# navigator8972/vae_assoc

Hardware: AMD Instinct MI355X
Metric: paired-samples/sec (img+jnt assoc-VAE train step) (higher is better)
Workload: dtype bf16

## Files before the change

### vae_assoc_amd/csrc/avae_device.h

```cpp
#pragma once
#include <hip/hip_runtime.h>
#include <math.h>
#include <stdint.h>
#include "../../include/avae.h"

namespace avae {

constexpr int kMaxMod = 4;
constexpr int kThreads = 256;
constexpr int kTileBytesK = 128;
constexpr int kRowAlign = 256;
constexpr int kLatentRows = 16;
constexpr int kAdamRows = 16;
constexpr int kCostHist = 4096;
constexpr int kSumsqThreads = 256;
constexpr int kSumsqMaxBlocks = 256;
constexpr int kSumsqQuads = 8;
inline int sumsq_blocks(long long p_int) {
    const long long quads = p_int / 4, per_block = (long long)kSumsqThreads * kSumsqQuads;
    const long long g = (quads + per_block - 1) / per_block;
    return (int)(g < 1 ? 1 : g > kSumsqMaxBlocks ? kSumsqMaxBlocks : g);
}
inline int sumsq_chain(long long p_int) {
    const long long quads = p_int / 4, per_pass = (long long)kSumsqThreads * sumsq_blocks(p_int);
    return (int)((quads + per_pass - 1) / per_pass);
}

enum Kind : int {
    K_FWD_HIDDEN = 0,
    K_FWD_HEAD = 1,
    K_FWD_OUT_LOSS = 2,
    K_FWD_OUT_STORE = 3,
    K_DGRAD_HIDDEN = 4,
    K_DGRAD_LATENT = 5,
    K_WGRAD = 6,
    K_DGRAD_F32 = 10,
    K_LATENT = 7,
    K_COST = 8,
    K_SERVE_Z = 11,
};

struct WorkItem {
    int kind;
    int M, N, K;
    int lda, ldb;
    int tiles_m, tiles_n;
    int act;
    int ld0, ld1, ldx;
    int nz;
    int binary;
    int ksplit, kchunk;
    int bias_row;
    int bias_ep;
    int kin;
    int tile_off, tile_cnt;
    int slot_base;
    int n_slots;
    int n_mod;
    int bump_step;
    float scale;
    float lambda;
    float inv_bg;
    const void* A;
    const void* B;
    void* out0;
    void* out1;
    void* out2;
    const void* aux0;
    const void* aux1;
    const void* aux2;
    float* partial;
    const float* eps;
    float wts[kMaxMod];
    const void* tail_w;
    void* tail_out;
    const void* tail_aux;
    int tail_mode;
    int tail_n;
    int tail_ldw, tail_ldo, tail_ldx;
    int tail_act;
    int tail_kt;
    int conv;
    const unsigned char* present;
    int present_ld;
};

struct ConvA {
    const void* src;
    const void* consts;
    int M, K;
    int OHW, OW, IH, IW, Cin;
    int k, so, d, pad;
    int src_sb, src_sp;
    int ones;
    unsigned mg_ohw, mg_ow, mg_k, mg_cin;
};
constexpr int kMaxConvA = 12;
constexpr int kMaxItemsPerLaunch = 12;
constexpr int kMaxPf = 4;
struct LaunchArgs {
    int n_items;
    int grid_x;
    int sched;
    int n_pf;
    const void* pf_ptr[4];
    int pf_lines[4];
    const ConvA* conv_tab;
    WorkItem items[kMaxItemsPerLaunch];
};

struct TnItem {
    const void* A;
    const void* B;
    float* out;
    int M, N, K;
    int lda, ldb, ld0;
    int tiles_m, tiles_n;
    int ksplit, kchunk;
    int bias_row;
    int tile_off, tile_cnt;
    int conv;
    void* W; void* Wt;
    int ldw, ldt;
};
constexpr int kMaxTnItems = 32;
constexpr int kTnPieces = 8;
struct TnPiece { unsigned short item, tile_off, cum_end, pad; };
struct DevState;
struct TnLaunchArgs {
    int n_items;
    int grid_x;
    int xcd_group;
    int sched;
    int adam;
    long long d_theta, d_m, d_v;
    float beta1, beta2, eps;
    const DevState* st;
    const ConvA* conv_tab;
    int xcd_pieces;
    TnPiece pieces[8][kTnPieces];
    TnItem items[kMaxTnItems];
};
static_assert(sizeof(TnLaunchArgs) <= 4096, "kernel arguments are passed by value: 4 KiB");

struct alignas(64) SmallDesc {
    const unsigned char* a;
    const unsigned char* b;
    void* out;
    const void* aux;
    int lda, ldb, ld0, ldx;
    int nk;
    int mrem, nrem, xrem;
};
struct alignas(64) TnDesc {
    const unsigned char* a;
    const unsigned char* b;
    float* out;
    void* w;
    void* wt;
    int lda, ldb, ld0, ldw, ldt;
    unsigned ext;
    static constexpr unsigned pack(int nk, int mrem, int nrem) { return (unsigned)nk | (unsigned)(mrem < 64 ? mrem : 64) << 16 | (unsigned)(nrem < 64 ? nrem : 64) << 24; }
};
static_assert(sizeof(SmallDesc) == 64 && sizeof(TnDesc) == 64, "a descriptor is one cache line");
struct DescWarm { const void* lines; int n; };
struct TnDescArgs {
    long long d_theta, d_m, d_v;
    float beta1, beta2, eps;
    const DevState* st;
};
constexpr int kTnDescHead = 8;
static_assert(sizeof(TnDescArgs) <= 64, "a copy of the constants is one line of the table");

struct DevState {
    long long step;
    float last_cost;
    float lr_t;
    float cost_hist[kCostHist];
};

struct ClipState {
    float max_norm;
    int skip_nonfinite;
    long long n_skipped;
    float partial[kSumsqMaxBlocks];
    float norm_hist[kCostHist];
};

struct EmaState {
    float decay;
    int warmup;
    int pad[30];
};
static_assert(sizeof(EmaState) == 128, "the average is line-aligned behind its settings");

struct HyperEntry { float kl, lambda, lr, pad; };
constexpr int kHyperSets = 16;
struct SchedState {
    avae_schedule sched[3];
    float lambda0, lr0;
    HyperEntry tab[kHyperSets];
    float hist[kCostHist][3];
};

__host__ __device__ inline float schedule_value(const avae_schedule& s, long long t) {
#pragma clang fp contract(off)
    long long u = t - 1;
    if (u < 0) u = 0;
    if (s.kind == AVAE_SCHED_PIECEWISE) {
        if (s.period > 0) u %= s.period;
        const int last = s.n_knots - 1;
        if (u <= s.knot_step[0]) return s.knot_value[0];
        if (u >= s.knot_step[last]) return s.knot_value[last];
        int i = 0;
        while (i + 1 < last && u >= s.knot_step[i + 1]) ++i;
        const double v0 = (double)s.knot_value[i], v1 = (double)s.knot_value[i + 1];
        const double f = (double)(u - s.knot_step[i]) / (double)(s.knot_step[i + 1] - s.knot_step[i]);
        return (float)(v0 + (v1 - v0) * f);
    }
    if (s.kind == AVAE_SCHED_EXP) {
        const double e = s.staircase ? (double)(u / s.decay_steps) : (double)u / (double)s.decay_steps;
        return (float)pow((double)s.decay_rate, e);
    }
    return 1.0f;
}

struct AdamItem {
    float* theta;
    float* m;
    float* v;
    const float* g;
    void* W;
    void* Wt;
    int rows, cols;
    int ld, ldt;
    int tiles_r, tiles_c, tile_base;
    int ldw;
    void* Wadj; void* Wf;
    int ldadj, ldf, adj_k, adj_cin;
};

constexpr int kMaxAdamItems = 80;
struct AdamArgs {
    const AdamItem* items;
    int n_items;
    int base[kMaxAdamItems];
    int mode;
    int book;
    float lr, beta1, beta2, eps;
    DevState* st;
    const float* cost_src;
    ClipState* clip;
    int n_partial;
    const EmaState* ema;
    float* avg;
    const float* theta0;
};

struct PrepSeg {
    const float* src; int src_ld;
    int rows, cols;
    float* dst32; int ld32;
    void* dstc; int ldc;
    int tiles_r, tiles_c, tile_base;
    const float* src_in; int in_ld;
    unsigned drop_thr;
    float drop_value, noise_std;
};
struct PrepArgs {
    PrepSeg seg[kMaxMod];
    int n_seg;
    int total_tiles;
    const float* eps_src;
    float* eps_dst;
    int eps_rows, nz, eps_blocks, eps_ld;
    int row_offset;
    unsigned long long seed;
    const DevState* st;
    unsigned long long stream_salt;
    int n_steps, blocks_per_step;
    long long set_stride;
    const unsigned char* pres_src;
    unsigned char* pres_dst;
    int pres_ld;
    int noisy;
    SchedState* sched;
};

struct ReduceSeg { float* dst; const float* src; int n, parts; long long stride; int block_base;
                   int dst_ld;
                   int colsum;
                   int perm_k, perm_cin, perm_cout, perm_ldga, perm_ld; };
constexpr int kMaxReduceSegs = 40;
struct ReduceArgs { ReduceSeg seg[kMaxReduceSegs]; int n_seg; };

struct ConvGeom {
    int B, IH, IW, Cin, OH, OW, k, so, d, pad;
    int src_sb, src_sp;
    int ones;
};
struct GatherSeg {
    ConvGeom g;
    const void* src;
    void* P; int ldp;
    int tiles_r, tiles_c, tile_base;
    int cl, rpt;
};
struct GatherArgs { GatherSeg seg[kMaxMod]; int n_seg; };
struct Col2imSeg {
    ConvGeom g;
    const float* dP; int lddp;
    const void* yprev; int ldy;
    int act;
    void* dA; int lda;
    const float* g0; int nz;
    const void* bias; int bias_ld;
    int tiles_r, tiles_c, tile_base;
// ... 33 lines not shown
void launch_gperm(const GpermArgs& a, int n_blocks, hipStream_t s);
struct RowsumSeg { const void* src; float* part; int ld, rows, cols, cols4, cpow, n_blocks, block_base; };
struct RowsumArgs { RowsumSeg seg[2 * kMaxMod]; int n_seg; };
void launch_rowsum(int compute_dtype, const RowsumArgs& a, int n_blocks, hipStream_t s);

struct ServeSlot {
    const float* z;
    float* out[kMaxMod];
    int rows;
    int pad;
};
struct ServeArgs {
    ServeSlot* slot;
    int n_mod, nz, bucket;
    void* Z[kMaxMod]; int ldz[kMaxMod];
    int blocks_per_mod;
};
void launch_serve(int compute_dtype, const ServeArgs& a, const ServeSlot& call, int n_blocks, hipStream_t s);
struct ServeInMod { const void* w; void* out; int n, ldw, ldo, kt, act, slices; };
struct ServeInArgs {
    ServeSlot call;
    ServeSlot* slot;
    int n_mod, nz, bucket, tiles_m;
    ServeInMod mod[kMaxMod];
};
void launch_serve_in(int compute_dtype, const ServeInArgs& a, int grid_x, hipStream_t s);

void launch_gather(int compute_dtype, const GatherArgs& a, int n_blocks, hipStream_t s);
void launch_col2im(int compute_dtype, const Col2imArgs& a, int n_blocks, hipStream_t s);

constexpr int kScoreRows = kThreads / 64;
struct ScoreLatentArgs {
    const float* mulv[kMaxMod];
    void* Z[kMaxMod]; int ldz[kMaxMod];
    const float* eps; int ld_eps;
    float* out; int k;
    int rows, nz, n_mod;
    int src;
    const unsigned char* present;
};
void launch_score_latent(int compute_dtype, const ScoreLatentArgs& a, hipStream_t s);
struct ScoreRowsArgs {
    const float* xhat; int ld32;
    const float* x; long long ldx;
    float* out; int k;
    int rows, n_in, binary, col;
    int cost;
    int n_mod, n_pair;
    float w[kMaxMod]; float lambda;
    const unsigned char* present; int pa, pb; unsigned absent_bits;
};
void launch_score_rows(const ScoreRowsArgs& a, hipStream_t s);

struct IwLatentArgs {
    const float* mulv;
    const float* eps;
    float* z32;
    void* Z[kMaxMod]; int ldz[kMaxMod]; int n_zdst;
    float* r;
    int rows, kc, k0, K, nz;
    long long row0;
    unsigned long long seed; unsigned draw;
    const unsigned char* present; int pres_ld;
};
void launch_iw_latent(int compute_dtype, const IwLatentArgs& a, hipStream_t s);
struct IwRowsArgs {
    const float* xhat[kMaxMod]; int ldh[kMaxMod];
    const float* x[kMaxMod]; long long ldx[kMaxMod];
    int n_in[kMaxMod], binary[kMaxMod];
    float* ell;
    int n_dec, kc, n_mod;
    const unsigned char* present;
};
void launch_iw_rows(const IwRowsArgs& a, hipStream_t s);
struct IwReduceArgs {
    const float* ell; const float* r;
    float* state;
    float* out; int width;
    int rows, kc, src, n_mod;
    int first, last;
    float log_k;
    const unsigned char* present;
};
void launch_iw_reduce(const IwReduceArgs& a, hipStream_t s);

struct ImputeFuseArgs {
    const float* mulv[kMaxMod];
    unsigned mods;
    const unsigned char* present;
    float* fused;
    float* mu; float* lv;
    float* z32;
    void* Z[kMaxMod]; int ldz[kMaxMod]; int n_zdst;
    int rows, nz, n_mod;
};
void launch_impute_fuse(int compute_dtype, const ImputeFuseArgs& a, hipStream_t s);
struct ImputeAccumArgs {
    const float* xhat[kMaxMod]; int ldh[kMaxMod];
    float* mean[kMaxMod]; float* var[kMaxMod];
    int n_in[kMaxMod];
    int tile0[kMaxMod + 1];
    int col0[kMaxMod];
    float* state; int ld_state;
    int rows, kc, k0, K, n_mod;
};
void launch_impute_accum(const ImputeAccumArgs& a, hipStream_t s);

constexpr int kMaxWorld = 8;
constexpr int kIpcThreads = 256;
struct IpcArgs {
    float* g;
    long long off, granules;
    long long cost_idx;
    int world, rank, wire_bf16, blocks;
    unsigned char* peer[kMaxWorld];
    long long off_flag1, off_flag2;
    long long off_cost;
    long long off_seq;
    long long off_err;
    long long off_slots, slot_stride, off_res;
    unsigned long long timeout_ticks;
};
void launch_ipc_allreduce(const IpcArgs& a, hipStream_t s);
void launch_wire_pack(const float* g, void* wire, long long n, hipStream_t s);
void launch_wire_unpack(float* g, const void* wire, long long n, hipStream_t s);

struct LaunchEvents { hipEvent_t start, stop; };
extern thread_local LaunchEvents t_launch_events;

constexpr int kStampLaunches = 32, kStampBlocks = 1024, kStampWords = 8;

int tile_lds_bytes(int tile_cfg, bool two_c_tiles);
void launch_grouped(int compute_dtype, int tile_cfg, const LaunchArgs& args, int grid_x, int grid_y, int lds_bytes,
                    DevState* st, hipStream_t s, unsigned long long* stamps = nullptr, int launch_id = 0);
void launch_grouped_tn(int compute_dtype, int tile_cfg, const TnLaunchArgs& args, int grid_x, int grid_y, int lds_bytes,
                       DevState* st, hipStream_t s, unsigned long long* stamps = nullptr, int launch_id = 0);
void launch_adam(int compute_dtype, const AdamArgs& a, int n_blocks, hipStream_t s);
void launch_grad_sumsq(const float* g, long long p_int, float* partial, hipStream_t s);
void launch_prep(int compute_dtype, const PrepArgs& a, hipStream_t s);
const void* prep_kernel(int compute_dtype, bool masked, bool noisy, bool sched);
void launch_fill(void* base, int elem_bytes, unsigned bits, long long start, long long stride, int count, hipStream_t s);
void launch_sums(const ReduceArgs& a, int n_blocks, hipStream_t s);
int small_head_lds_bytes();
void launch_small_latb(int compute_dtype, int act, const LaunchArgs& args, int grid_x, int grid_y, int lds_bytes, DevState* st, hipStream_t s,
                       unsigned long long* stamps, int launch_id);
void launch_small_head(int compute_dtype, int act, const LaunchArgs& args, int grid_x, int grid_y, int lds_bytes, hipStream_t s,
                       unsigned long long* stamps, int launch_id);
void launch_small_tn(int compute_dtype, const TnLaunchArgs& args, int grid_x, int grid_y, hipStream_t s, unsigned long long* stamps, int launch_id);
void launch_small_loss(int compute_dtype, const LaunchArgs& args, int grid_x, int grid_y, int lds_bytes, hipStream_t s, unsigned long long* stamps, int launch_id);
void launch_small(int compute_dtype, const LaunchArgs& args, int grid_x, int grid_y, int lds_bytes, hipStream_t s, unsigned long long* stamps, int launch_id);
void launch_small_desc(int compute_dtype, bool dgrad, int act, const SmallDesc* tab, int n_tiles, int lds_bytes, DescWarm warm, hipStream_t s,
                       unsigned long long* stamps, int launch_id);
void launch_small_tn_desc(int compute_dtype, const TnDesc* tab, int n_tiles, DescWarm warm, hipStream_t s, unsigned long long* stamps, int launch_id);
void launch_reduce(const ReduceArgs& a, int n_blocks, hipStream_t s);
void launch_chain2(int compute_dtype, const LaunchArgs& args, int grid_x, int grid_y, int lds_bytes, unsigned* counters, unsigned* err, hipStream_t s);

}
```

### vae_assoc_amd/csrc/avae_host.hip

```cpp
#include "avae_device.h"
#include "avae_complete.h"
#include "avae_retrieve.h"
#include "avae_latent_stats.h"
#include "avae_gmm.h"
#include "avae_embed.h"
#include "avae_aggpost.h"
#include "../../include/avae.h"

#include <dlfcn.h>
#include <sched.h>
#include <unistd.h>

#include <algorithm>
#include <cctype>
#include <cstddef>
#include <cmath>
#include <cstdio>
#include <cstdlib>
#include <cstring>
#include <functional>
#include <map>
#include <mutex>
#include <stdexcept>
#include <string>
// ... 1815 lines not shown
    } else if (md.conv) {
        for (int i = 0; i < 4; ++i) {
            if (md.cdec[i].dense_map) {
                Launch L;
                L.name = "inf_conv_dec_direct"; L.type = 4;
                L.ta.mode = 0;
                ThinSeg t = bd.thin_seg(md.cdec[i], md.cdec[i - 1]);
                t.block_base = 0;
                L.ta.seg[0] = t; L.ta.n_seg = 1;
                L.blocks = rows * t.split;
                inf.launches.push_back(L);
                continue;
            }
            gather1(md.cdec[i], i == 0 ? h->at<void>(md.Z.rm) : h->at<void>(md.cdec[i - 1].Y.rm), "inf_conv_im2col");
            one(bd.conv_fwd(md.cdec[i]), "inf_conv_dec");
        }
        if (!md.cdec[3].dense_map) gather1(md.cdec[4], h->at<void>(md.cdec[3].Y.rm), "inf_conv_im2col");
        one(bd.fwd_out(md, m, false), "inf_out");
    } else {
        for (int k = 0; k < md.L; ++k) one(bd.fwd_hidden(k == 0 ? md.Z : md.D[k - 1], md.dec[k], md.D[k]), "inf_dec");
        one(bd.fwd_out(md, m, false), "inf_out");
    }
    inf.rows = rows;
}

int tname_id(avae_handle* h, const std::string& n) {
    for (size_t i = 0; i < h->tnames.size(); ++i) if (h->tnames[i] == n) return (int)i;
    h->tnames.push_back(n);
    return (int)h->tnames.size() - 1;
}

struct Timed {
    avae_handle* h; hipStream_t s; bool on; hipEvent_t a = nullptr, b = nullptr; int id = 0;
    Timed(avae_handle* h_, hipStream_t s_, const std::string& name) : h(h_), s(s_), on(h_->timing && h_->trecs.size() < 200000) {
        if (!on) return;
        id = tname_id(h, name);
        HIP_OK(hipEventCreate(&a)); HIP_OK(hipEventCreate(&b));
        t_launch_events = LaunchEvents{a, b};
    }
    ~Timed() {
        if (!on) return;
        if (t_launch_events.start) {
            t_launch_events = LaunchEvents{nullptr, nullptr};
            (void)hipEventRecord(a, s); (void)hipEventRecord(b, s);
        }
        h->trecs.push_back(TimingRec{a, b, id});
    }
};

template <typename F> void timed_launch(avae_handle* h, hipStream_t s, const char* name, F&& launch) {
    Timed t(h, s, name);
    launch();
    LAUNCH_OK(name);
}

Launch relocated(const avae_handle* h, const Launch& L0, int j, const HyperEntry* hyper = nullptr) {
    Launch L = L0;
    const unsigned char* lo = h->ws + h->stage_lo;
    const unsigned char* hi = lo + h->stage_bytes;
    const size_t delta = (size_t)j * h->stage_bytes;
    auto fix = [&](auto& ptr) {
        const unsigned char* q = reinterpret_cast<const unsigned char*>(ptr);
        if (q >= lo && q < hi) ptr = reinterpret_cast<std::remove_reference_t<decltype(ptr)>>(const_cast<unsigned char*>(q) + delta);
    };
    for (int i = 0; i < L.args.n_items && L.type == 0; ++i) {
        WorkItem& w = L.args.items[i];
        fix(w.A); fix(w.B); fix(w.out0); fix(w.out1); fix(w.out2); fix(w.aux0); fix(w.aux1); fix(w.aux2); fix(w.eps);
        fix(w.tail_w); fix(w.tail_out); fix(w.tail_aux);
        if (w.present) w.present += (size_t)j * h->pres_set;
        if (hyper && (w.kind == K_LATENT || (w.kind == K_COST && w.bump_step))) w.tail_w = hyper + j;
    }
    for (int i = 0; i < L.targs.n_items && L.type == 0; ++i) { TnItem& t = L.targs.items[i]; fix(t.A); fix(t.B); fix(t.out); }
    for (int i = 0; i < L.ga.n_seg && L.type == 1; ++i) fix(L.ga.seg[i].src);
    L.desc_set = j;
    return L;
}

template <typename D> std::vector<D> deal_to_xcds(const std::vector<D> (&lists)[8]) {
    size_t total = 0;
    for (const auto& l : lists) total += l.size();
    std::vector<D> out(total), spill;
    std::vector<char> set(total, 0);
    for (int p = 0; p < 8; ++p)
        for (size_t i = 0; i < lists[p].size(); ++i) {
            const size_t x = 8 * i + p;
            if (x < total) { out[x] = lists[p][i]; set[x] = 1; } else spill.push_back(lists[p][i]);
        }
    size_t k = 0;
    for (size_t x = 0; x < total; ++x) if (!set[x]) out[x] = spill[k++];
    return out;
}

std::vector<SmallDesc> small_descs(const avae_handle* h, const Launch& L) {
    std::vector<SmallDesc> lists[8];
    const int es = h->es;
    for (int y = 0; y < L.args.n_items; ++y) {
        const WorkItem& w = L.args.items[y];
        if (w.kind != L.args.items[0].kind || w.act != L.args.items[0].act || (w.kind != K_FWD_HIDDEN && w.kind != K_DGRAD_HIDDEN)) return {};
        const int nt = w.tiles_m * w.tiles_n, q = nt >> 3, r = nt & 7;
        for (int part = 0; part < 8; ++part)
            for (int idx = 0; idx < q + (part < r ? 1 : 0); ++idx) {
                const int t = (part < r ? part * (q + 1) : r * (q + 1) + (part - r) * q) + idx;
                const int tm = t / w.tiles_n, tn = t - tm * w.tiles_n, m0 = tm * 32, n0 = tn * 32;
                SmallDesc d{};
                d.a = static_cast<const unsigned char*>(w.A) + (size_t)m0 * w.lda * es;
                d.b = static_cast<const unsigned char*>(w.B) + (size_t)n0 * w.ldb * es;
                d.out = static_cast<unsigned char*>(w.out0) + ((size_t)m0 * w.ld0 + n0) * es;
                d.aux = w.kind == K_DGRAD_HIDDEN ? static_cast<const unsigned char*>(w.aux0) + ((size_t)m0 * w.ldx + n0) * es : nullptr;
                d.lda = w.lda; d.ldb = w.ldb; d.ld0 = w.ld0; d.ldx = w.ldx;
                d.nk = (w.K * es) / kTileBytesK;
                d.mrem = w.M - m0; d.nrem = w.N - n0; d.xrem = w.ldx - n0;
                lists[part].push_back(d);
            }
    }
    return deal_to_xcds(lists);
}

std::vector<TnDesc> tn_descs(const avae_handle* h, const Launch& L) {
    std::vector<TnDesc> lists[8];
    const TnLaunchArgs& a = L.targs;
    const int es = h->es;
    for (int y = 0; y < L.grid_y; ++y)
        for (int x = 0; x < L.grid_x; ++x) {
            const int part = x & 7, idx = x >> 3;
            int entry = y, t = -1;
            if (a.xcd_pieces) {
                int e = 0, lo = 0;
                for (int i = 0; i < kTnPieces; ++i) { const int ce = a.pieces[part][i].cum_end; if (idx >= ce) { e = i + 1; lo = ce; } }
                if (e >= kTnPieces) continue;
                entry = a.pieces[part][e].item; t = a.pieces[part][e].tile_off + idx - lo;
            } else {
                if (entry >= a.n_items) continue;
                const int nt = a.items[entry].tile_cnt, q = nt >> 3, r = nt & 7;
                if (idx >= q + (part < r ? 1 : 0)) continue;
                t = (part < r ? part * (q + 1) : r * (q + 1) + (part - r) * q) + idx + a.items[entry].tile_off;
            }
            const TnItem& w = a.items[entry];
            const int tm = t / w.tiles_n, tn = t - tm * w.tiles_n, m0 = tm * 64, n0 = tn * 64;
            const int nk = (w.K * es) / kTileBytesK;
            if (nk > 65535 || !w.W || !w.Wt) return {};
            TnDesc d{};
            d.a = static_cast<const unsigned char*>(w.A) + (size_t)m0 * es;
            d.b = static_cast<const unsigned char*>(w.B) + (size_t)n0 * es;
            d.out = w.out + (size_t)m0 * w.ld0 + n0;
            d.w = static_cast<unsigned char*>(w.W) + ((size_t)m0 * w.ldw + n0) * es;
            d.wt = static_cast<unsigned char*>(w.Wt) + ((size_t)n0 * w.ldt + m0) * es;
            d.lda = w.lda; d.ldb = w.ldb; d.ld0 = w.ld0; d.ldw = w.ldw; d.ldt = w.ldt;
            d.ext = TnDesc::pack(nk, w.M - m0, w.N - n0);
            lists[part].push_back(d);
        }
    return deal_to_xcds(lists);
}

void build_descriptors(avae_handle* h, hipStream_t s) {
    if (std::getenv("AVAE_NO_DESC")) return;
    std::vector<unsigned char> tab;
    auto add = [&](Launch& L) {
        if (L.type != 0 || !((L.cfg == 7 && !L.tn) || (L.cfg == 12 && L.tn && L.targs.adam))) return;
        const size_t off = tab.size();
        size_t stride = 0;
        int n = 0;
        for (int j = 0; j < kMultiSteps; ++j) {
            const Launch Lj = j == 0 ? L : relocated(h, L, j);
            const size_t at = tab.size();
            if (L.tn) {
                const std::vector<TnDesc> d = tn_descs(h, Lj);
                if (d.empty()) { tab.resize(off); return; }
                const TnDescArgs ca = {L.targs.d_theta, L.targs.d_m, L.targs.d_v, L.targs.beta1, L.targs.beta2, L.targs.eps, L.targs.st};
                tab.resize(at + (kTnDescHead + d.size()) * 64, 0);
                for (int p = 0; p < kTnDescHead; ++p) std::memcpy(tab.data() + at + 64 * p, &ca, sizeof(ca));
                std::memcpy(tab.data() + at + 64 * kTnDescHead, d.data(), d.size() * 64);
                n = (int)d.size();
            } else {
                const std::vector<SmallDesc> d = small_descs(h, Lj);
                if (d.empty()) { tab.resize(off); return; }
                tab.resize(at + d.size() * 64);
                std::memcpy(tab.data() + at, d.data(), d.size() * 64);
                n = (int)d.size();
            }
            stride = tab.size() - at;
        }
        L.desc_n = n; L.desc_off = off; L.desc_stride = stride;
    };
    for (Launch& L : h->plain.fwd) add(L);
    for (Launch& L : h->bwd) add(L);
    for (Launch& L : h->wgrad_adam) add(L);
    if (tab.empty()) return;
    HIP_OK(hipMemcpyAsync(h->desc_buf.ensure(tab.size()), tab.data(), tab.size(), hipMemcpyHostToDevice, s));
    HIP_OK(hipStreamSynchronize(s));
}

template <typename D> const D* desc_of(const avae_handle* h, const Launch& L) {
    return reinterpret_cast<const D*>(h->desc_buf.as<unsigned char>() + L.desc_off + (size_t)L.desc_set * L.desc_stride);
}

DescWarm warm_for(const avae_handle* h, const Launch* next, int next_set) {
    if (!next || next->desc_n == 0 || next_set >= kMultiSteps) return DescWarm{nullptr, 0};
    return DescWarm{h->desc_buf.as<unsigned char>() + next->desc_off + (size_t)next_set * next->desc_stride,
                    next->desc_n + (next->tn ? kTnDescHead : 0)};
}

void dump_launch(const Launch& L) {
    std::fprintf(stderr, "[avae] launch %s type=%d cfg=%d items=%d blocks=%d\n", L.name.c_str(), L.type, L.cfg, L.count, L.blocks);
    if (L.desc_n) std::fprintf(stderr, "        descriptors=%d set=%d\n", L.desc_n, L.desc_set);
    for (int i = 0; i < L.args.n_items && L.type == 0; ++i)
        std::fprintf(stderr, "        item kind=%d M=%d N=%d K=%d lda=%d ldb=%d tiles=%dx%d\n", L.args.items[i].kind, L.args.items[i].M,
                     L.args.items[i].N, L.args.items[i].K, L.args.items[i].lda, L.args.items[i].ldb, L.args.items[i].tiles_m, L.args.items[i].tiles_n);
    for (int i = 0; i < L.ga.n_seg && L.type == 1; ++i)
        std::fprintf(stderr, "        gather B=%d IH=%d Cin=%d OH=%d k=%d so=%d d=%d pad=%d sb=%d sp=%d ones=%d ldp=%d tiles=%dx%d\n", L.ga.seg[i].g.B, L.ga.seg[i].g.IH,
                     L.ga.seg[i].g.Cin, L.ga.seg[i].g.OH, L.ga.seg[i].g.k, L.ga.seg[i].g.so, L.ga.seg[i].g.d, L.ga.seg[i].g.pad, L.ga.seg[i].g.src_sb, L.ga.seg[i].g.src_sp,
                     L.ga.seg[i].g.ones, L.ga.seg[i].ldp, L.ga.seg[i].tiles_r, L.ga.seg[i].tiles_c);
    for (int i = 0; i < L.ca.n_seg && L.type == 2; ++i)
        std::fprintf(stderr, "        col2im B=%d IH=%d Cin=%d OH=%d k=%d lddp=%d lda=%d g0=%p tiles=%dx%d\n", L.ca.seg[i].g.B, L.ca.seg[i].g.IH, L.ca.seg[i].g.Cin,
                     L.ca.seg[i].g.OH, L.ca.seg[i].g.k, L.ca.seg[i].lddp, L.ca.seg[i].lda, (const void*)L.ca.seg[i].g0, L.ca.seg[i].tiles_r, L.ca.seg[i].tiles_c);
}

void run_launch(avae_handle* h, const Launch& L, hipStream_t s, unsigned long long* stamps, int stamp, DescWarm warm = DescWarm{nullptr, 0}) {
    Timed t(h, s, L.name);
    if (L.type == 1) launch_gather(h->cfg.compute_dtype, L.ga, L.blocks, s);
    else if (L.type == 2) launch_col2im(h->cfg.compute_dtype, L.ca, L.blocks, s);
    else if (L.type == 3) launch_reduce(L.ra, L.blocks, s);
    else if (L.type == 4) launch_thin(h->cfg.compute_dtype, L.ta, L.blocks, s);
    else if (L.type == 5) launch_colsum(L.ra, L.blocks, s);
    else if (L.type == 6) launch_wadj(h->cfg.compute_dtype, L.wa, L.blocks, s);
    else if (L.type == 7) launch_gperm(L.gp, L.blocks, s);
    else if (L.type == 8) launch_rowsum(h->cfg.compute_dtype, L.rs, L.blocks, s);
    else if (L.type == 9) launch_sums(L.ra, L.blocks, s);
    else if (L.cfg == 13) launch_chain2(h->cfg.compute_dtype, L.args, L.grid_x, L.grid_y, L.lds, h->at<unsigned>(h->off_chain), h->at<unsigned>(h->off_chain) + kMaxMod * 64, s);
    else if (L.cfg == 11) launch_small_head(h->cfg.compute_dtype, L.lean_act, L.args, L.grid_x, L.grid_y, L.lds, s, stamps, stamp);
    else if (L.cfg == 10) launch_small_latb(h->cfg.compute_dtype, L.lean_act, L.args, L.grid_x, L.grid_y, L.lds, h->state(), s, stamps, stamp);
    else if (L.cfg == 9) launch_small_loss(h->cfg.compute_dtype, L.args, L.grid_x, L.grid_y, L.lds, s, stamps, stamp);
    else if (L.cfg == 7 && L.desc_n) launch_small_desc(h->cfg.compute_dtype, L.args.items[0].kind == K_DGRAD_HIDDEN, L.args.items[0].act, desc_of<SmallDesc>(h, L), L.desc_n, L.lds, warm, s, stamps, stamp);
    else if (L.cfg == 7) launch_small(h->cfg.compute_dtype, L.args, L.grid_x, L.grid_y, L.lds, s, stamps, stamp);
    else if (L.tn && L.cfg == 12 && L.desc_n) launch_small_tn_desc(h->cfg.compute_dtype, desc_of<TnDesc>(h, L), L.desc_n, warm, s, stamps, stamp);
    else if (L.tn && L.cfg == 12) launch_small_tn(h->cfg.compute_dtype, L.targs, L.grid_x, L.grid_y, s, stamps, stamp);
    else if (L.tn) launch_grouped_tn(h->cfg.compute_dtype, L.cfg, L.targs, L.grid_x, L.grid_y, L.lds, h->state(), s, stamps, stamp);
    else launch_grouped(h->cfg.compute_dtype, L.cfg, L.args, L.grid_x, L.grid_y, L.lds, h->state(), s, stamps, stamp);
    LAUNCH_OK(L.name);
    if (h->debug_sync) {
        dump_launch(L);
        std::fflush(stderr);
        HIP_OK(hipStreamSynchronize(s));
    }
}

bool has_hyper_item(const Launch& L) {
    for (int i = 0; i < L.args.n_items && L.type == 0; ++i)
        if (L.args.items[i].kind == K_LATENT || (L.args.items[i].kind == K_COST && L.args.items[i].bump_step)) return true;
    return false;
}

void run_set(avae_handle* h, const std::vector<Launch>& ls, size_t lo, size_t hi, int j, hipStream_t s, int stamp_base = -1, bool train = false,
             const Launch* after = nullptr, int after_set = 0) {
    unsigned long long* stamps = nullptr;
#ifdef AVAE_STAMPS
    if (stamp_base >= 0) stamps = h->at<unsigned long long>(h->off_stamps);
#endif
    const HyperEntry* hyper = nullptr;
    if (train && h->sched_on) {
        if (!h->sched_buf.p) throw Err("internal error: a schedule is on without its device state");
        if (j < 0 || j >= kHyperSets) throw Err("internal error: staging set outside the schedule table");
        hyper = h->sched_buf.as<SchedState>()->tab;
    }
    for (size_t i = lo; i < hi && i < ls.size(); ++i) {
        const int k = stamp_base + (int)(i - lo);
        const bool last = i + 1 >= hi || i + 1 >= ls.size();
        const DescWarm warm = last ? warm_for(h, after, after_set) : warm_for(h, &ls[i + 1], j);
        if (j == 0 && !(hyper && has_hyper_item(ls[i]))) run_launch(h, ls[i], s, stamps, k, warm);
        else run_launch(h, relocated(h, ls[i], j, hyper), s, stamps, k, warm);
    }
}

void run_launches(avae_handle* h, const std::vector<Launch>& ls, hipStream_t s) { run_set(h, ls, 0, ls.size(), 0, s); }

void run_adam(avae_handle* h, int mode, hipStream_t s, int bucket = -1, bool from_avg = false) {
    AdamArgs a;
    std::memset(&a, 0, sizeof(a));
    int blocks = h->adam_blocks;
    if (bucket < 0) {
        a.items = h->at<AdamItem>(h->off_adam);
        a.n_items = (int)h->adam_items.size();
        if (a.n_items > kMaxAdamItems) throw Err("internal error: too many Adam items");
        for (int i = 0; i < a.n_items; ++i) a.base[i] = h->adam_items[i].tile_base;
    } else {
        a.items = h->at<AdamItem>(h->off_adam_b) + h->adam_first_b[bucket];
        a.n_items = h->adam_count_b[bucket];
        for (int i = 0; i < a.n_items; ++i) a.base[i] = h->adam_items_b[h->adam_first_b[bucket] + i].tile_base;
        blocks = h->adam_blocks_b[bucket];
        if (blocks == 0) return;
    }
    a.book = (bucket <= 0) ? 1 : 0;
    a.mode = mode;
    a.lr = h->cfg.learning_rate; a.beta1 = h->cfg.beta1; a.beta2 = h->cfg.beta2; a.eps = h->cfg.adam_eps;
    a.st = h->state();
    a.cost_src = h->grad() + h->P_int;
    a.clip = (mode == 0 && h->clip_on) ? h->clip_buf.as<ClipState>() : nullptr;
    a.n_partial = sumsq_blocks((long long)h->P_int);
    if (mode == 0 ? h->ema_on : from_avg) {
        if (!h->ema_buf.p) throw Err("internal error: averaging is on without its device state");
        a.ema = h->ema_buf.as<EmaState>(); a.avg = h->ema_avg(); a.theta0 = h->at<float>(h->off_theta);
    }
    Timed t(h, s, mode == 0 ? (bucket < 0 ? "adam" : bucket == 0 ? "adam_dec" : "adam_enc") : "shadow_refresh");
    launch_adam(h->cfg.compute_dtype, a, blocks, s);
    LAUNCH_OK(mode == 0 ? "adam" : "shadow_refresh");
}

void run_grad_sumsq(avae_handle* h, hipStream_t s) {
    ClipState* cs = h->clip_buf.as<ClipState>();
    if (!cs) throw Err("internal error: clipping is on without its device state");
    timed_launch(h, s, "grad_sumsq", [&] { launch_grad_sumsq(h->grad(), (long long)h->P_int, cs->partial, s); });
}

struct PrepIn { const float* const* in = nullptr; const int32_t* in_ld = nullptr; bool corrupt = false; };

PrepArgs new_prep(const avae_handle* h, unsigned long long salt, int row0 = 0) {
    PrepArgs a;
    std::memset(&a, 0, sizeof(a));
    a.row_offset = h->cfg.row_offset + row0; a.seed = h->cfg.seed; a.st = h->state(); a.stream_salt = salt;
    return a;
}

int fill_prep_seg(const avae_handle* h, PrepSeg& g, const float* src, int src_ld, int rows, int cols, const Act& dst, float* dst32,
                  int ld32, int tile_base) {
    g.src = src; g.src_ld = src_ld; g.rows = rows; g.cols = cols;
    g.dst32 = dst32; g.ld32 = ld32;
    g.dstc = h->at<void>(dst.rm); g.ldc = dst.ld;
    g.tiles_r = (rows + 63) / 64; g.tiles_c = (cols + 63) / 64; g.tile_base = tile_base;
    return g.tiles_r * g.tiles_c;
}

void fill_prep_eps(const avae_handle* h, PrepArgs& a, const float* eps, int rows) {
    a.eps_src = eps; a.eps_dst = h->at<float>(h->off_eps); a.eps_rows = rows; a.nz = h->nz; a.eps_ld = h->ld_eps;
    a.eps_blocks = (rows * ((h->nz + 3) / 4) + kThreads - 1) / kThreads;
}

PrepArgs make_prep_batch(avae_handle* h, const float* const* x, const int32_t* x_ld, const float* eps, int rows,
                         unsigned long long salt, int n_steps = 1, const uint8_t* present = nullptr, const PrepIn& pin = PrepIn()) {
    PrepArgs a = new_prep(h, salt);
    int base = 0;
    for (int m = 0; m < h->M; ++m) {
        const Mod& md = h->mods[m];
        PrepSeg& g = a.seg[m];
        base += fill_prep_seg(h, g, x[m], (x_ld && x_ld[m] > 0) ? x_ld[m] : md.n_in, rows, md.n_in, md.X0, h->at<float>(md.X32), md.ld32, base);
        if (pin.in && pin.in[m]) {
            g.src_in = pin.in[m]; g.in_ld = (pin.in_ld && pin.in_ld[m] > 0) ? pin.in_ld[m] : md.n_in;
            a.noisy = 1;
        } else if (pin.corrupt && (h->drop_thr[m] != 0u || h->corr.noise_std[m] > 0.0f)) {
            g.drop_thr = h->drop_thr[m]; g.drop_value = h->corr.drop_value[m]; g.noise_std = h->corr.noise_std[m];
            a.noisy = 1;
        }
    }
    a.n_seg = h->M; a.total_tiles = base;
    fill_prep_eps(h, a, eps, rows);
    a.n_steps = n_steps; a.blocks_per_step = a.total_tiles + a.eps_blocks; a.set_stride = (long long)h->stage_bytes;
    if (present) { a.pres_src = present; a.pres_dst = h->pres_buf.as<unsigned char>(); a.pres_ld = h->M; }
    if (h->sched_on && salt == kTrainSalt) a.sched = h->sched_buf.as<SchedState>();
    return a;
}

void run_prep_batch(avae_handle* h, const float* const* x, const int32_t* x_ld, const float* eps, int rows,
                    unsigned long long salt, hipStream_t s, const uint8_t* present = nullptr, int n_steps = 1, const PrepIn& pin = PrepIn()) {
    const PrepArgs a = make_prep_batch(h, x, x_ld, eps, rows, salt, n_steps, present, pin);
    timed_launch(h, s, "prep", [&] { launch_prep(h->cfg.compute_dtype, a, s); });
}

struct PrepOne {
    const float* src; int src_ld, rows, cols;
    const Act& dst;
    int row0;
    PrepOne(const float* src_, int src_ld_, int rows_, int cols_, const Act& dst_, int row0_ = 0)
        : src(src_), src_ld(src_ld_), rows(rows_), cols(cols_), dst(dst_), row0(row0_) {}
    float* dst32 = nullptr; int ld32 = 0;
    bool eps = false;
    const float* eps_src = nullptr;
    unsigned long long salt = 0;
    PrepOne& with_eps(const float* e, unsigned long long salt_ = 0) { eps = true; eps_src = e; salt = salt_; return *this; }
    const unsigned char* pres_src = nullptr; unsigned char* pres_dst = nullptr; int pres_ld = 0;
};

void run_prep_single(avae_handle* h, const PrepOne& p, hipStream_t s) {
    PrepArgs a = new_prep(h, p.salt, p.row0);
    if (p.pres_src) { a.pres_src = p.pres_src; a.pres_dst = p.pres_dst; a.pres_ld = p.pres_ld; }
    if (p.src || p.pres_src) {
        a.n_seg = 1;
        a.total_tiles = fill_prep_seg(h, a.seg[0], p.src, p.src_ld, p.rows, p.cols, p.dst, p.dst32, p.ld32, 0);
    }
    if (p.eps) fill_prep_eps(h, a, p.eps_src, p.rows);
    launch_prep(h->cfg.compute_dtype, a, s);
    LAUNCH_OK("prep");
}

StepGraph capture(avae_handle* h, const std::function<void(hipStream_t)>& body, bool with_prep = false) {
    StepGraph sg;
    const bool tsave = h->timing;
    h->timing = false;
    HIP_OK(hipStreamBeginCapture(h->cap_stream, hipStreamCaptureModeThreadLocal));
    try { body(h->cap_stream); }
    catch (...) { (void)hipStreamEndCapture(h->cap_stream, &sg.graph); sg.release(); h->timing = tsave; throw; }
    h->timing = tsave;
    HIP_OK(hipStreamEndCapture(h->cap_stream, &sg.graph));
    try {
        if (with_prep) {
            size_t n_root = 0;
            HIP_OK(hipGraphGetRootNodes(sg.graph, nullptr, &n_root));
            if (n_root != 1) throw Err("internal error: the captured step is not a chain");
            HIP_OK(hipGraphGetRootNodes(sg.graph, &sg.prep, &n_root));
            hipGraphNodeType ty;
            HIP_OK(hipGraphNodeGetType(sg.prep, &ty));
            if (ty != hipGraphNodeTypeKernel) throw Err("internal error: the captured step does not start with the staging kernel");
        }
        HIP_OK(hipGraphInstantiate(&sg.exec, sg.graph, nullptr, nullptr, 0));
        if (!with_prep) { HIP_OK(hipGraphDestroy(sg.graph)); sg.graph = nullptr; }
    } catch (...) { sg.release(); throw; }
    return sg;
}

void patch_prep(avae_handle* h, const StepGraph& sg, const float* const* x, const int32_t* x_ld, const float* eps,
                int n_steps, const uint8_t* present, const PrepIn& pin) {
    PrepArgs a = make_prep_batch(h, x, x_ld, eps, h->B, kTrainSalt, n_steps, present, pin);
    void* kp[1] = {&a};
    hipKernelNodeParams np;
    std::memset(&np, 0, sizeof(np));
    np.func = const_cast<void*>(prep_kernel(h->cfg.compute_dtype, present != nullptr, a.noisy != 0, a.sched != nullptr));
    np.gridDim = dim3((a.total_tiles + a.eps_blocks) * n_steps); np.blockDim = dim3(kThreads);
    np.sharedMemBytes = 0; np.kernelParams = kp; np.extra = nullptr;
    HIP_OK(hipGraphExecKernelNodeSetParams(sg.exec, sg.prep, &np));
}

void fill_ones(avae_handle* h, const Act& a, hipStream_t s) {
    if (!a.ones) return;
    const unsigned bits = h->es == 2 ? 0x3F80u : 0x3F800000u;
    launch_fill(h->at<void>(a.rm), h->es, bits, a.width, a.ld, h->B, s);
    LAUNCH_OK("fill");
}

void step_body(avae_handle* h, const std::vector<Launch>& fwd, hipStream_t s, int j, int stamp_base = -1, bool more = false) {
    auto sb = [&](size_t k) { return stamp_base < 0 ? -1 : stamp_base + (int)k; };
    auto first_of = [](const std::vector<Launch>& ls) { return ls.empty() ? nullptr : &ls[0]; };
    const bool fused = !h->wgrad_adam.empty() && !h->clip_on && !h->ema_on;
    run_set(h, fwd, 0, fwd.size(), j, s, stamp_base, true, first_of(h->bwd), j);
    run_set(h, h->bwd, 0, h->bwd.size(), j, s, sb(fwd.size()), true, fused ? first_of(h->wgrad_adam) : nullptr, j);
    if (fused) {
        run_set(h, h->wgrad_adam, 0, h->wgrad_adam.size(), j, s, sb(fwd.size() + h->bwd.size()), true, more ? first_of(fwd) : nullptr, j + 1);
        return;
    }
    run_set(h, h->wgrad, 0, h->wgrad.size(), j, s, sb(fwd.size() + h->bwd.size()), true);
    if (h->clip_on) run_grad_sumsq(h, s);
    run_adam(h, 0, s);
}

void capture_steps(avae_handle* h, StepPlan& p, const uint8_t* present) {
    std::vector<const float*> x0(h->M, h->at<float>(h->mods[0].X32));
    try {
        p.full = capture(h, [&](hipStream_t cs) {
            run_prep_batch(h, x0.data(), nullptr, nullptr, h->B, kTrainSalt, cs, present);
            step_body(h, p.fwd, cs, 0, 0);
        }, true);
        for (int gi = 0; gi < 2; ++gi) p.multi[gi] = capture(h, [&](hipStream_t cs) {
            run_prep_batch(h, x0.data(), nullptr, nullptr, h->B, kTrainSalt, cs, present, kMultiSizes[gi]);
            for (int j = 0; j < kMultiSizes[gi]; ++j) step_body(h, p.fwd, cs, j, -1, j + 1 < kMultiSizes[gi]);
        }, true);
    } catch (...) { p.full.release(); p.multi[0].release(); p.multi[1].release(); throw; }
}

void capture_plan(avae_handle* h, StepPlan& p, const uint8_t* present) {
    try {
        capture_steps(h, p, present);
        p.eval = capture(h, [&](hipStream_t cs) { run_launches(h, p.fwd, cs); run_launch(h, h->cost_only, cs, nullptr, -1); });
    } catch (...) { p.release(); throw; }
}

void init_device(avae_handle* h) {
    hipStream_t s = h->cap_stream;
    HIP_OK(hipMemsetAsync(h->ws, 0, h->ws_bytes, s));
    for (const Mod& md : h->mods) {
        for (int j = 0; j < kMultiSteps; ++j) {
            Act x = md.X0;
            x.rm += (size_t)j * h->stage_bytes;
            fill_ones(h, x, s);
        }
        for (const Act& a : md.E) fill_ones(h, a, s);
        fill_ones(h, md.Z, s);
        for (const Act& a : md.D) fill_ones(h, a, s);
        if (md.conv && md.cdec[3].dense_map) fill_ones(h, md.cdec[3].Y, s);
    }
    build_training_plan(h);
    build_descriptors(h, s);
    HIP_OK(hipMemcpyAsync(h->at<void>(h->off_adam), h->adam_items.data(), h->adam_items.size() * sizeof(AdamItem), hipMemcpyHostToDevice, s));
    HIP_OK(hipMemcpyAsync(h->at<void>(h->off_adam_b), h->adam_items_b.data(), h->adam_items_b.size() * sizeof(AdamItem), hipMemcpyHostToDevice, s));
    {
        static const unsigned char c32_bf16[32] = {0, 0, 0, 0, 0, 0, 0, 0, 0, 0, 0, 0, 0, 0, 0, 0, 0x80, 0x3F};
        static const unsigned char c32_f32[32] = {0, 0, 0, 0, 0, 0, 0, 0, 0, 0, 0, 0, 0, 0, 0, 0, 0, 0, 0x80, 0x3F};
        HIP_OK(hipMemcpyAsync(h->at<void>(h->off_consts), h->es == 2 ? c32_bf16 : c32_f32, 32, hipMemcpyHostToDevice, s));
        if (!h->conv_tab.empty()) {
            const unsigned char* lo = h->ws + h->stage_lo;
            for (const ConvA& c : h->conv_tab)
                if (reinterpret_cast<const unsigned char*>(c.src) >= lo && reinterpret_cast<const unsigned char*>(c.src) < lo + h->stage_bytes * kMultiSteps)
                    throw Err("internal error: an implicit patch matrix on a staged input (not relocatable per step)");
            HIP_OK(hipMemcpyAsync(h->at<void>(h->off_conv_tab), h->conv_tab.data(), h->conv_tab.size() * sizeof(ConvA), hipMemcpyHostToDevice, s));
        }
    }
    size_t off = h->off_inf;
    h->inf_enc.assign(h->M, avae_handle::Inf());
    h->inf_dec.assign(h->M, avae_handle::Inf());
    for (int m = 0; m < h->M; ++m) {
        h->inf_enc[m].dev_off = off; off += ((size_t)h->mods[m].L + 1) * sizeof(WorkItem);
        h->inf_dec[m].dev_off = off; off += ((size_t)h->mods[m].L + 1) * sizeof(WorkItem);
    }
    HIP_OK(hipStreamSynchronize(s));
    if (h->cfg.use_graph) capture_plan(h, h->plain, nullptr);
}

void comm_check_error(avae_handle* h);

void fetch_cost(avae_handle* h, float* cost_host, bool from_state, hipStream_t s) {
    if (!cost_host) return;
    const void* src = from_state ? (const void*)&h->state()->last_cost : (const void*)(h->grad() + h->P_int);
    HIP_OK(hipMemcpyAsync(cost_host, src, sizeof(float), hipMemcpyDeviceToHost, s));
    HIP_OK(hipStreamSynchronize(s));
    comm_check_error(h);
}

void copy_rows(void* dst, size_t dpitch, const void* src, size_t spitch, size_t width, size_t rows, hipStream_t s) {
    HIP_OK(hipMemcpy2DAsync(dst, dpitch, src, spitch, width, rows, hipMemcpyDeviceToDevice, s));
}

hipStream_t on_stream(avae_handle* h, void* stream) {
    hipStream_t s = reinterpret_cast<hipStream_t>(stream);
    if (h->has_last_stream && s != h->last_stream) {
        if (!h->ev_switch) HIP_OK(hipEventCreateWithFlags(&h->ev_switch, hipEventDisableTiming));
        if (hipEventRecord(h->ev_switch, h->last_stream) == hipSuccess) HIP_OK(hipStreamWaitEvent(s, h->ev_switch, 0));
        else (void)hipGetLastError();
    }
    h->last_stream = s; h->has_last_stream = true;
    return s;
}

void check_schedule(const avae_schedule& c, const std::string& who) {
    auto fail = [&](const std::string& what) { throw Err(who + ": " + what); };
    if (c.kind == AVAE_SCHED_NONE) return;
    if (c.kind == AVAE_SCHED_PIECEWISE) {
        if (c.n_knots < 1 || c.n_knots > AVAE_SCHED_MAX_KNOTS)
            fail("n_knots = " + std::to_string(c.n_knots) + " must be in [1, " + std::to_string(AVAE_SCHED_MAX_KNOTS) + "]");
        if (c.period < 0) fail("period = " + std::to_string((long long)c.period) + " must be >= 0");
        for (int i = 0; i < c.n_knots; ++i) {
            if (i == 0 ? c.knot_step[0] < 0 : c.knot_step[i] <= c.knot_step[i - 1])
                fail("knot_step[" + std::to_string(i) + "] = " + std::to_string((long long)c.knot_step[i]) +
                     (i == 0 ? " must be >= 0" : " must be above knot_step[" + std::to_string(i - 1) + "] (strictly increasing)"));
            if (!(c.knot_value[i] >= 0.0f) || std::isinf(c.knot_value[i]))
                fail("knot_value[" + std::to_string(i) + "] must be finite and >= 0");
        }
        if (c.period > 0 && c.knot_step[c.n_knots - 1] >= c.period)
            fail("knot_step[" + std::to_string(c.n_knots - 1) + "] = " + std::to_string((long long)c.knot_step[c.n_knots - 1]) +
                 " must be below period = " + std::to_string((long long)c.period));
        return;
    }
    if (c.kind == AVAE_SCHED_EXP) {
        if (!(c.decay_rate > 0.0f) || std::isinf(c.decay_rate)) fail("decay_rate must be finite and > 0");
        if (c.decay_steps <= 0) fail("decay_steps = " + std::to_string((long long)c.decay_steps) + " must be > 0");
        if (c.staircase != 0 && c.staircase != 1) fail("staircase must be 0 or 1");
        return;
    }
    fail("kind = " + std::to_string(c.kind) + " is none of AVAE_SCHED_NONE, AVAE_SCHED_PIECEWISE, AVAE_SCHED_EXP");
}

avae_schedule canonical_schedule(const avae_schedule& c) {
    avae_schedule o;
    std::memset(&o, 0, sizeof(o));
    o.kind = c.kind;
    if (c.kind == AVAE_SCHED_PIECEWISE) {
        o.n_knots = c.n_knots; o.period = c.period;
        for (int i = 0; i < c.n_knots; ++i) { o.knot_step[i] = c.knot_step[i]; o.knot_value[i] = c.knot_value[i]; }
    } else if (c.kind == AVAE_SCHED_EXP) {
        o.decay_rate = c.decay_rate; o.staircase = c.staircase; o.decay_steps = c.decay_steps;
    }
    return o;
}

template <typename F> int guarded(avae_handle* h, F&& f) {
    if (!h) return 1;
    std::lock_guard<std::mutex> lk(h->mu);
    try {
        DeviceGuard dg(h->cfg.device);
        f();
        return 0;
    } catch (const std::exception& e) {
        h->err = e.what();
        return 2;
    }
}

void master_to_host(avae_handle* h, size_t off, std::vector<float>& host) {
    host.resize(h->P_int);
    HIP_OK(hipDeviceSynchronize());
// ... 385 lines not shown
void stage_and_encode(avae_handle* h, const RowInputs& in, const RowPresence& pres, int r0, int n, bool encode_null,
                      const StageEps* eps, hipStream_t s) {
    for (int m = 0; m < h->M; ++m) {
        if (!in.x[m] && !pres) continue;
        const Mod& md = h->mods[m];
        PrepOne p(in.at(m, r0), in.ld[m], n, md.n_in, md.X0, r0);
        if (eps && m == 0) p.with_eps(eps->src ? eps->src + (size_t)r0 * h->nz : nullptr);
        if (eps) p.salt = eps->salt;
        if (pres) { p.pres_src = pres.src + (size_t)r0 * h->M + m; p.pres_dst = pres.staged + m; p.pres_ld = h->M; }
        run_prep_single(h, p, s);
        if (in.x[m] || encode_null) run_inference(h, m, true, n, s);
    }
}

struct DecodeAll {
    avae_handle* h;
    bool by_mod;
    explicit DecodeAll(avae_handle* h_) : h(h_), by_mod(decode_by_mod(h_)) {}
    template <typename Args> void z_dest(Args& a, float* z32) const {
        if (!by_mod) { a.z32 = z32; return; }
        a.n_zdst = h->M;
        for (int m = 0; m < h->M; ++m) { a.Z[m] = h->at<void>(h->mods[m].Z.rm); a.ldz[m] = h->mods[m].Z.ld; }
    }
    int ld_out32(int m) const { return by_mod ? h->mods[m].ld32 : h->mods[m].n_in; }
    void run(int nd, const float* z, bool stage_z, float* const* dst, bool dst_only, hipStream_t s) const {
        if (by_mod) {
            for (int m = 0; m < h->M; ++m) {
                float* out = dst ? dst[m] : nullptr;
                if (dst_only && !out) continue;
                if (stage_z) { decode_rows(h, m, z, nd, out, s); continue; }
                run_inference(h, m, false, nd, s);
                if (out) copy_out32(h, m, out, nd, s);
            }
            return;
        }
        ServeSlot sl;
        std::memset(&sl, 0, sizeof(sl));
        for (int c0 = 0; c0 < nd; c0 += h->B) {
            sl.z = z + (size_t)c0 * h->nz; sl.rows = std::min(h->B, nd - c0);
            for (int m = 0; m < h->M; ++m)
                sl.out[m] = (dst && dst[m]) ? dst[m] + (size_t)c0 * h->mods[m].n_in : h->at<float>(h->mods[m].out32);
            serve_call(h, serve_plan(h, serve_bucket(h, sl.rows)), sl, s);
        }
    }
};

struct SampleBlocks {
    int K, n_rows, kb;
    SampleBlocks(int K_, int cap) : K(K_), n_rows(K_ >= cap ? 1 : cap / std::max(K_, 1)), kb(K_ >= cap ? cap : K_) {}
    template <typename F> void each(int nj, F&& body) const {
        for (int k0 = 0; k0 < K; k0 += kb) {
            const int kc = std::min(kb, K - k0);
            body(k0, kc, nj * kc);
        }
    }
};

constexpr int kCompleteSizes[3] = {16, 4, 1};

void complete_pass(avae_handle* h, avae_handle::Complete& cp, hipStream_t s) {
    run_launches(h, cp.fwd, s);
    timed_launch(h, s, "complete_out", [&] { launch_complete_out(h->cfg.compute_dtype, cp.args, s); });
    run_launches(h, cp.bwd, s);
    timed_launch(h, s, "complete_update", [&] { launch_complete_update(h->cfg.compute_dtype, cp.args, s); });
}

avae_handle::Complete& complete_plan(avae_handle* h) {
    avae_handle::Complete& cp = h->cmpl;
    if (cp.built) return cp;
    const int B = h->B, M = h->M, nz = h->nz, lddz = (int)rup(nz, 4);
    Bump b;
    const size_t off_call = b.take(sizeof(CompleteCall));
    const size_t off_z = b.take((size_t)B * nz * 4), off_m = b.take((size_t)B * nz * 4), off_v = b.take((size_t)B * nz * 4);
    const size_t off_recon = b.take((size_t)B * M * 4);
    size_t off_dz[kMaxMod] = {0, 0, 0, 0};
    for (int m = 0; m < M; ++m) off_dz[m] = b.take(rup(B, kRowAlign) * (size_t)lddz * 4);
    unsigned char* buf = static_cast<unsigned char*>(cp.buf.ensure(b.off, true));
    CompleteArgs& a = cp.args;
    std::memset(&a, 0, sizeof(a));
    a.call = reinterpret_cast<CompleteCall*>(buf + off_call);
    a.z32 = reinterpret_cast<float*>(buf + off_z); a.m = reinterpret_cast<float*>(buf + off_m); a.v = reinterpret_cast<float*>(buf + off_v);
    a.recon = reinterpret_cast<float*>(buf + off_recon);
    a.beta1 = h->cfg.beta1; a.beta2 = h->cfg.beta2; a.eps = h->cfg.adam_eps;
    a.n_mod = M; a.nz = nz; a.bucket = B;
    for (int m = 0; m < M; ++m) {
        const Mod& md = h->mods[m];
        a.Z[m] = h->at<void>(md.Z.rm); a.ldz[m] = md.Z.ld;
        a.out32[m] = h->at<float>(md.out32); a.ld32[m] = md.ld32;
        a.dO[m] = h->at<void>(md.dO.rm); a.lddo[m] = md.dO.ld;
        a.dz[m] = reinterpret_cast<float*>(buf + off_dz[m]); a.lddz[m] = lddz;
        a.n_in[m] = md.n_in; a.binary[m] = h->cfg.mod[m].binary ? 1 : 0; a.w[m] = h->cfg.mod[m].weight;
    }
    cp.items.clear(); cp.fwd.clear(); cp.bwd.clear();
    Builder bd(h, cp.items, B, false);
    Groups group{h, cp.items};
    int Lmax = 0;
    for (const Mod& md : h->mods) Lmax = std::max(Lmax, md.L);
    for (int k = 0; k < Lmax; ++k)
        group("cmpl_dec" + std::to_string(k + 1), cp.fwd, [&] {
            for (Mod& md : h->mods) if (k < md.L) cp.items.push_back(bd.fwd_hidden(k == 0 ? md.Z : md.D[k - 1], md.dec[k], md.D[k])); });
    group("cmpl_out", cp.fwd, [&] { for (int m = 0; m < M; ++m) cp.items.push_back(bd.fwd_out(h->mods[m], m, false)); });
    group("cmpl_bwd_out", cp.bwd, [&] {
        for (Mod& md : h->mods) cp.items.push_back(bd.dgrad_hidden(md.dO, md.outl, md.D.back(), md.dD.back())); });
    for (int k = Lmax - 1; k >= 1; --k)
        group("cmpl_bwd_dec" + std::to_string(k + 1), cp.bwd, [&] {
            for (Mod& md : h->mods) if (k < md.L) cp.items.push_back(bd.dgrad_hidden(md.dD[k], md.dec[k], md.D[k - 1], md.dD[k - 1])); });
    group("cmpl_bwd_dz", cp.bwd, [&] {
        for (int m = 0; m < M; ++m) {
            const Mod& md = h->mods[m];
            const Dense& d = md.dec[0];
            WorkItem w = gemm_item(K_DGRAD_F32, B, nz, bd.K_of(d.out), h->at<void>(md.dD[0].rm), md.dD[0].ld, h->at<void>(d.W), d.ldw);
            w.out0 = const_cast<float*>(a.dz[m]); w.ld0 = lddz;
            cp.items.push_back(w);
        } });
    if (h->cfg.use_graph) {
        try {
            for (int i = 0; i < 3; ++i)
                cp.g[i] = capture(h, [&](hipStream_t cs) { for (int j = 0; j < kCompleteSizes[i]; ++j) complete_pass(h, cp, cs); });
        } catch (...) { for (StepGraph& g : cp.g) g.release(); throw; }
    }
    cp.built = true;
    return cp;
}

void build_masked(avae_handle* h) {
    if (!h->masked.fwd.empty()) return;
    h->pres_set = (size_t)h->B * h->M;
    unsigned char* pres = static_cast<unsigned char*>(h->pres_buf.ensure(h->pres_set * kMultiSteps, true));
    std::vector<Launch> mf = h->plain.fwd;
    int n_loss = 0, n_latent = 0;
    for (Launch& L : mf) {
        if (L.type != 0 || L.tn) continue;
        bool gated = false;
        for (int i = 0; i < L.args.n_items; ++i) {
            WorkItem& w = L.args.items[i];
            if (w.kind == K_FWD_OUT_LOSS) {
                int m = 0;
                while (m < h->M && w.aux0 != h->at<void>(h->mods[m].X32)) ++m;
                if (m == h->M) throw Err("internal error: a loss item of no modality");
                w.present = pres + m; w.present_ld = h->M;
                gated = true; ++n_loss;
            } else if (w.kind == K_LATENT) {
                w.present = pres; w.present_ld = h->M;
                gated = true; ++n_latent;
            }
        }
        const int c = L.cfg;
        if (gated && !(c == 0 || c == 1 || c == 3 || c == 4 || c == 5 || c == 6 || c == 9))
            throw Err("masked training is not available on this plan: launch " + L.name + " (tile configuration " + std::to_string(c) +
                      ") carries a loss or latent item on a kernel without the presence gate");
    }
    if (n_loss != h->M || n_latent != 1) throw Err("internal error: the masked twin found " + std::to_string(n_loss) + " loss and " +
                                                   std::to_string(n_latent) + " latent items");
    h->masked.fwd.swap(mf);
    if (h->cfg.use_graph) {
        try { capture_plan(h, h->masked, pres); } catch (...) { h->masked.fwd.clear(); throw; }
    }
}

void check_masked_call(avae_handle* h, const char* what, const float* const* x_dev, const uint8_t* present_dev) {
    if (h->cfg.world_size > 1 || h->cfg.use_comm != AVAE_COMM_NONE || h->comm_on)
        throw Err(std::string(what) + ": masked steps run on one replica only (world_size 1, use_comm AVAE_COMM_NONE)");
    if (!x_dev) throw Err(std::string(what) + ": null x_dev");
    if (!present_dev) throw Err(std::string(what) + ": present_dev is null (unmasked calls go through the unmasked entry points)");
}

void check_inputs(avae_handle* h, const char* what, const float* const* x_dev, const float* const* in_dev, const int32_t* in_ld) {
    if (!x_dev) throw Err(std::string(what) + ": null x_dev");
    for (int m = 0; in_dev && m < h->M; ++m) {
        if (!in_dev[m]) continue;
        if (!x_dev[m]) throw Err(std::string(what) + ": in_dev[" + std::to_string(m) + "] is set while x_dev[" + std::to_string(m) + "] is null");
        if (in_ld && in_ld[m] > 0 && in_ld[m] < h->mods[m].n_in)
            throw Err(std::string(what) + ": in_ld[" + std::to_string(m) + "] = " + std::to_string(in_ld[m]) + " is below n_input = " +
                      std::to_string(h->mods[m].n_in));
    }
}

void train_one(avae_handle* h, StepPlan& p, const float* const* x_dev, const int32_t* x_ld, const uint8_t* present, const float* eps_dev,
               const PrepIn& pin, hipStream_t s) {
    if (h->comm_on) {
        run_prep_batch(h, x_dev, x_ld, eps_dev, h->B, kTrainSalt, s, nullptr, 1, pin);
        dp_step(h, 0, s);
        return;
    }
    if (p.full.exec && !h->timing) {
        patch_prep(h, p.full, x_dev, x_ld, eps_dev, 1, present, pin);
        HIP_OK(hipGraphLaunch(p.full.exec, s));
        return;
    }
    run_prep_batch(h, x_dev, x_ld, eps_dev, h->B, kTrainSalt, s, present, 1, pin);
    step_body(h, p.fwd, s, 0);
    if (h->timing) {
        timed_launch(h, s, "_null_kernel", [&] { launch_fill(h->at<void>(h->off_partial), 4, 0u, 0, 1, 1, s); });
    }
}

struct BatchRun {
    const avae_handle* h;
    const float* const* x_dev;
    const int32_t* x_ld;
    const uint8_t* present;
    const float* eps_dev;
    const float* const* in_dev;
    const int32_t* in_ld;
    const float* x[kMaxMod] = {};
    const float* in[kMaxMod] = {};
    const uint8_t* pres = nullptr;
    const float* eps = nullptr;
    PrepIn pin() const { return PrepIn{in, in_ld, true}; }
    void at(int i) {
        for (int m = 0; m < h->M; ++m) {
            const size_t ld = (x_ld && x_ld[m] > 0) ? (size_t)x_ld[m] : (size_t)h->mods[m].n_in;
            x[m] = x_dev[m] ? x_dev[m] + (size_t)i * h->B * ld : nullptr;
            const size_t ldi = (in_ld && in_ld[m] > 0) ? (size_t)in_ld[m] : (size_t)h->mods[m].n_in;
            in[m] = (in_dev && in_dev[m]) ? in_dev[m] + (size_t)i * h->B * ldi : nullptr;
        }
        pres = present ? present + (size_t)i * h->B * h->M : nullptr;
        eps = eps_dev ? eps_dev + (size_t)i * h->B * h->nz : nullptr;
    }
};

template <typename Ready>
int replay_runs(avae_handle* h, StepGraph (&g)[2], BatchRun& b, int n_steps, hipStream_t s, Ready&& ready) {
    int i = 0;
    for (int gi = 0; gi < 2; ++gi)
        for (; i + kMultiSizes[gi] <= n_steps && ready(gi); i += kMultiSizes[gi]) {
            b.at(i);
            patch_prep(h, g[gi], b.x, b.x_ld, b.eps, kMultiSizes[gi], b.pres, b.pin());
            HIP_OK(hipGraphLaunch(g[gi].exec, s));
        }
    return i;
}

void train_steps(avae_handle* h, StepPlan& p, int n_steps, const float* const* x_dev, const int32_t* x_ld, const float* const* in_dev,
                 const int32_t* in_ld, const uint8_t* present, const float* eps_dev, float* cost_host, hipStream_t s) {
    BatchRun b{h, x_dev, x_ld, present, eps_dev, in_dev, in_ld};
    int i = 0;
    if (h->comm_on) {
        if (h->cfg.use_graph && !h->timing)
            i = replay_runs(h, h->g_dpm, b, n_steps, s, [&](int gi) {
                if (h->dp_graph_failed) return false;
                if (h->g_dpm[gi].exec) return true;
                std::vector<const float*> x0(h->M, h->at<float>(h->mods[0].X32));
                try {
                    h->g_dpm[gi] = capture(h, [&](hipStream_t cs) {
                        run_prep_batch(h, x0.data(), nullptr, nullptr, h->B, kTrainSalt, cs, nullptr, kMultiSizes[gi]);
                        for (int j = 0; j < kMultiSizes[gi]; ++j) dp_step(h, j, cs, true);
                    }, true);
                } catch (const std::exception& e) {
                    h->dp_graph_failed = true;
                    (void)hipGetLastError();
                    if (std::getenv("AVAE_DEBUG_DP")) std::fprintf(stderr, "[avae] data-parallel graph capture failed (%s): host-stepped pipeline\n", e.what());
                    return false;
                }
                return true;
            });
        for (; i < n_steps; i += kMultiSteps) {
            const int n = std::min(kMultiSteps, n_steps - i);
            b.at(i);
            run_prep_batch(h, b.x, x_ld, b.eps, h->B, kTrainSalt, s, nullptr, n, b.pin());
            for (int j = 0; j < n; ++j) dp_step(h, j, s);
        }
    } else {
        if (!h->timing) i = replay_runs(h, p.multi, b, n_steps, s, [&](int gi) { return p.multi[gi].exec != nullptr; });
        for (; i < n_steps; ++i) {
            b.at(i);
            train_one(h, p, b.x, x_ld, b.pres, b.eps, b.pin(), s);
        }
    }
    if (h->clip_on) h->clip_steps += n_steps;
    if (h->sched_on) h->sched_steps += n_steps;
    fetch_cost(h, cost_host, true, s);
}

void eval_cost(avae_handle* h, StepPlan& p, const float* const* x_dev, const int32_t* x_ld, const float* const* in_dev, const int32_t* in_ld,
               const uint8_t* present, const float* eps_dev, float* cost_host, hipStream_t s) {
    run_prep_batch(h, x_dev, x_ld, eps_dev, h->B, 0x6576616cull  | (unsigned long long)next_draw(h, eps_dev) << 34, s, present, 1,
                   PrepIn{in_dev, in_ld, false});
    if (p.eval.exec && !h->timing) HIP_OK(hipGraphLaunch(p.eval.exec, s));
    else { run_launches(h, p.fwd, s); run_launch(h, h->cost_only, s, nullptr, -1); }
    fetch_cost(h, cost_host, false, s);
}

void require_live(const avae_handle* h, const char* who) {
    if (h->averaged)
        throw Err(std::string(who) + ": the handle runs on the averaged weights; call avae_use_averaged(h, 0) before training");
}

void ema_to_host(avae_handle* h, std::vector<float>& host) {
    host.resize(h->P_int);
    HIP_OK(hipDeviceSynchronize());
    HIP_OK(hipMemcpy(host.data(), h->ema_avg(), h->P_int * 4, hipMemcpyDeviceToHost));
}
void host_to_ema(avae_handle* h, const std::vector<float>& host) {
    HIP_OK(hipDeviceSynchronize());
    HIP_OK(hipMemcpy(h->ema_avg(), host.data(), h->P_int * 4, hipMemcpyHostToDevice));
}
void ema_from_theta(avae_handle* h) {
    HIP_OK(hipDeviceSynchronize());
    HIP_OK(hipMemcpy(h->ema_avg(), h->at<void>(h->off_theta), h->P_int * 4, hipMemcpyDeviceToDevice));
    HIP_OK(hipDeviceSynchronize());
}

void use_averaged(avae_handle* h, bool on) {
    if (on && !h->ema_on) throw Err("avae_use_averaged: parameter averaging is off (avae_set_ema)");
    if (on == h->averaged) return;
// ... 1487 lines not shown
```

### vae_assoc_amd/csrc/avae_kernels.hip

```cpp
#include "avae_device.h"
#include "avae_complete.h"
#include <hip/hip_ext.h>
#include <stdexcept>
#include "../../include/avae.h"

namespace avae {

typedef __attribute__((ext_vector_type(8))) __bf16 bf16x8;
typedef __attribute__((ext_vector_type(4))) __bf16 bf16x4;
typedef __attribute__((ext_vector_type(4))) float f32x4;
typedef __attribute__((ext_vector_type(4))) unsigned u32x4;


template <typename CT> __device__ __forceinline__ CT to_ct(float v);
template <> __device__ __forceinline__ float to_ct<float>(float v) { return v; }
template <> __device__ __forceinline__ __bf16 to_ct<__bf16>(float v) { return (__bf16)v; }

__device__ __forceinline__ float bf16_bits_to_float(unsigned b) { return __uint_as_float(b << 16); }

template <typename CT> __device__ __forceinline__ void load4(const CT* p, float v[4]);
template <> __device__ __forceinline__ void load4<float>(const float* p, float v[4]) {
    float4 t = *reinterpret_cast<const float4*>(p);
    v[0] = t.x; v[1] = t.y; v[2] = t.z; v[3] = t.w;
}
// ... 1125 lines not shown
                for (int k = 0; k < HALF; ++k) {
                    if (rws[k] < BM) {
#pragma unroll
                        for (int e = 0; e < 4; ++e) {
                            const int d = 4 * qs[k] + e;
                            if (d < nz) {
                                const float dz = Cs[cs_idx<LDC>(rws[k], d)];
                                Zs[cs_idx<LDC>(rws[k], d)] = dz + gm[k][e];
                                Zs[cs_idx<LDC>(rws[k], nz + d)] = __builtin_fmaf(dz, gf[k][e], gl[k][e]);
                            }
                        }
                    }
                }
            }
        }
        lds_barrier();
        if (ts == 0)
            tile_pass<CT, CT, false, false, BM, BN>(Zs, reinterpret_cast<CT*>(w.out0), w.ld0, (const CT*)nullptr, 8,
                                                    M, 2 * nz, m0, 0, [](float c, float, bool) { return c; });
        if (tail_on) { t_src = Zs; t_cols = 2 * nz; t_one = -1; }
      }
    } break;
    case K_SERVE_Z: {
      if constexpr (TAIL) {
        const int nz = w.nz, rows = w.n_slots;
        float* Zs = Cs + BM * LDC;
        const float* zsrc = reinterpret_cast<const float*>(w.aux0);
        for (int i = tid; i < BM * nz; i += NT) {
            const int r = i / nz, d = i - r * nz;
            Zs[cs_idx<LDC>(r, d)] = m0 + r < rows ? zsrc[(size_t)(m0 + r) * nz + d] : 0.0f;
        }
        if (blockIdx.x == 0 && blockIdx.y == 0 && tid == 0) {
            ServeSlot* sp = reinterpret_cast<ServeSlot*>(w.partial);
            sp->z = zsrc; sp->rows = rows;
            sp->out[0] = reinterpret_cast<float*>(w.out0); sp->out[1] = reinterpret_cast<float*>(w.out1);
            sp->out[2] = reinterpret_cast<float*>(w.out2); sp->out[3] = reinterpret_cast<float*>(const_cast<void*>(w.aux1));
        }
        lds_barrier();
        if (tail_on) { t_src = Zs; t_cols = nz; t_one = nz; }
      }
    } break;
    case K_DGRAD_F32:
    case K_WGRAD: {
        float* G = reinterpret_cast<float*>(w.out0);
        tile_pass<float, float, false, false, BM, BN, NT>(Cs, G, w.ld0, (const float*)nullptr, 4, M, N, m0, n0,
            [](float c, float, bool) { return c; });
    } break;
    default: break;
    }
    if (t_src) tail_product(t_src, t_cols, t_one);
    AVAE_STAMP(4)
    AVAE_STAMP_FLUSH()
    return;
    }
    if constexpr (!TN && (NW == 4 || (NW == 8 && BN == 64))) {
        if (w.kind == K_LATENT) latent_item<NW, MASK>(w, t, red);
        else cost_item<NW>(w, st, red);
        AVAE_STAMP(4)
        AVAE_STAMP_FLUSH()
    }
}

template <typename CT, int KIND, int ACT>
__global__ void __launch_bounds__(kThreads) k_small(const LaunchArgs args, unsigned long long* stamps, int launch_id) {
    constexpr int BM = 32, RING = 4, ES = (int)sizeof(CT), NCH = 2;
    constexpr int kStage = 64 * kTileBytesK;
    unsigned char* smem = avae_dyn_smem;
#ifdef AVAE_STAMPS
    unsigned long long sv[kStampWords] = {0, 0, 0, 0, 0, 0, 0, 0};
#endif
    AVAE_STAMP(0)
    const int part = blockIdx.x & 7, idx = blockIdx.x >> 3;
    const WorkItem w = args.items[blockIdx.y];
    asm volatile("" :: "s"(w.A), "s"(w.B), "s"(w.out0), "s"(w.aux0), "s"(w.lda), "s"(w.ldb), "s"(w.K), "s"(w.ld0), "s"(w.ldx));
    int t;
    {
        const int nt = w.tiles_m * w.tiles_n;
        const int q = nt >> 3, r = nt & 7;
        if (idx >= q + (part < r ? 1 : 0)) return;
        t = (part < r ? part * (q + 1) : r * (q + 1) + (part - r) * q) + idx;
    }
    const int tid = threadIdx.x, lane = tid & 63, wave = __builtin_amdgcn_readfirstlane(tid >> 6);
    const int wr = wave >> 1, wc = wave & 1, fr = lane & 15, fq = lane >> 4;
    const int tm = t / w.tiles_n, tn = t - tm * w.tiles_n;
    const int m0 = tm * BM, n0 = tn * 32;
    const int nk = (w.K * ES) / kTileBytesK;
    typedef const __attribute__((address_space(1))) void* gp_t;
    typedef __attribute__((address_space(3))) void* lp_t;
    const int prow = wave * 8 + (lane >> 3), lc = ((lane & 7) ^ ((prow >> 1) & 7)) * 16;
    const unsigned char* srcA = reinterpret_cast<const unsigned char*>(w.A) + (size_t)(m0 + prow) * w.lda * ES + lc;
    const unsigned char* srcB = reinterpret_cast<const unsigned char*>(w.B) + (size_t)(n0 + prow) * w.ldb * ES + lc;
    const int orow = m0 + wr * 16 + fr, ocol = n0 + wc * 16 + 4 * fq;
    typename Quad<CT>::raw yq;
    if constexpr (KIND == 1)
        yq = *reinterpret_cast<const typename Quad<CT>::raw*>(reinterpret_cast<const CT*>(w.aux0) + (size_t)min(orow, w.M - 1) * w.ldx + min(ocol, w.ldx - 4));
#define AVAE_S_DMA(kt, buf)                                                                                             \
    { __builtin_amdgcn_global_load_lds((gp_t)(srcA + (size_t)(kt) * kTileBytesK), (lp_t)(smem + (buf) * kStage + wave * 1024), 16, 0, 0);          \
      __builtin_amdgcn_global_load_lds((gp_t)(srcB + (size_t)(kt) * kTileBytesK), (lp_t)(smem + (buf) * kStage + (4 + wave) * 1024), 16, 0, 0); }
    AVAE_STAMP(1)
    const int npro = nk < RING - 1 ? nk : RING - 1;
    for (int p = 0; p < npro; ++p) AVAE_S_DMA(p, p)
    const int sw0 = (fq ^ (fr >> 1)) * 16;
    const int aoff = (wr * 16 + fr) * kTileBytesK, boff = (32 + wc * 16 + fr) * kTileBytesK;
    f32x4 acc = {0.f, 0.f, 0.f, 0.f};
    int buf = 0;
    for (int kt = 0; kt < nk; ++kt) {
        const int rem = nk - 1 - kt;
        if (rem >= 2) asm volatile("s_waitcnt vmcnt(4)" ::: "memory");
        else if (rem == 1) asm volatile("s_waitcnt vmcnt(2)" ::: "memory");
        else asm volatile("s_waitcnt vmcnt(0)" ::: "memory");
        asm volatile("s_barrier" ::: "memory");
        if (kt == 0) { AVAE_STAMP(2) }
        const unsigned char* Sb = smem + buf * kStage;
        const u32x4 a0 = *reinterpret_cast<const u32x4*>(Sb + aoff + sw0), b0 = *reinterpret_cast<const u32x4*>(Sb + boff + sw0);
        const int fill = buf == 0 ? RING - 1 : buf - 1;
        if (kt + RING - 1 < nk) AVAE_S_DMA(kt + RING - 1, fill)
        const u32x4 a1 = *reinterpret_cast<const u32x4*>(Sb + aoff + (sw0 ^ 64)), b1 = *reinterpret_cast<const u32x4*>(Sb + boff + (sw0 ^ 64));
        mma<CT>(b0, a0, acc);
        mma<CT>(b1, a1, acc);
        buf = buf + 1 == RING ? 0 : buf + 1;
    }
#undef AVAE_S_DMA
    AVAE_STAMP(3)
    if constexpr (KIND == 2) {
        float v[4];
#pragma unroll
        for (int e = 0; e < 4; ++e) v[e] = w.binary ? sigmoidf_(acc[e]) : acc[e];
        if (w.aux2) {
            const ServeSlot* sp = reinterpret_cast<const ServeSlot*>(w.aux2);
            float* dst = sp->out[w.n_mod] + (size_t)orow * w.N + ocol;
            if (orow < sp->rows) {
#pragma unroll
                for (int e = 0; e < 4; ++e) if (ocol + e < w.N) dst[e] = v[e];
            }
        } else if (orow < w.M && ocol < w.N) {
            store_row<float>(reinterpret_cast<float*>(w.out0) + (size_t)orow * w.ld0 + ocol, v, w.N - ocol);
        }
    } else if (orow < w.M && ocol < w.N) {
        float v[4];
#pragma unroll
        for (int e = 0; e < 4; ++e) {
            if constexpr (KIND == 0) v[e] = act_fwd_t<ACT>(acc[e]);
            else v[e] = acc[e] * act_bwd_t<ACT>(quad_elem<CT>(yq, e));
        }
        store_row<CT>(reinterpret_cast<CT*>(w.out0) + (size_t)orow * w.ld0 + ocol, v, w.N - ocol);
    }
    AVAE_STAMP(4)
    AVAE_STAMP_FLUSH()
}

__device__ __forceinline__ unsigned desc_warm(const void* lines, int n, int wave) {
    typedef const __attribute__((address_space(4))) unsigned* cu_t;
    const int i = (blockIdx.x & 7) + 8 * (4 * (blockIdx.x >> 3) + wave);
    return i < n ? *(cu_t)((unsigned long long)lines + 64ull * (unsigned)i) : 0u;
}

template <typename CT, int KIND, int ACT>
__global__ void __launch_bounds__(kThreads) k_small_desc(const SmallDesc* __restrict__ tab, unsigned long long* stamps, int launch_id,
                                                         const void* warm_lines, int warm_n) {
    constexpr int RING = 4, ES = (int)sizeof(CT);
    constexpr int kStage = 64 * kTileBytesK;
    unsigned char* smem = avae_dyn_smem;
#ifdef AVAE_STAMPS
    unsigned long long sv[kStampWords] = {0, 0, 0, 0, 0, 0, 0, 0};
#endif
    AVAE_STAMP(0)
    const SmallDesc d = tab[blockIdx.x];
    const int tid = threadIdx.x, lane = tid & 63, wave = __builtin_amdgcn_readfirstlane(tid >> 6);
    const int wr = wave >> 1, wc = wave & 1, fr = lane & 15, fq = lane >> 4;
    const int nk = d.nk;
    typedef const __attribute__((address_space(1))) void* gp_t;
    typedef __attribute__((address_space(3))) void* lp_t;
    const int prow = wave * 8 + (lane >> 3), lc = ((lane & 7) ^ ((prow >> 1) & 7)) * 16;
    const unsigned char* srcA = d.a + (size_t)prow * d.lda * ES + lc;
    const unsigned char* srcB = d.b + (size_t)prow * d.ldb * ES + lc;
    const int lrow = wr * 16 + fr, lcol = wc * 16 + 4 * fq;
    typename Quad<CT>::raw yq;
    if constexpr (KIND == 1)
        yq = *reinterpret_cast<const typename Quad<CT>::raw*>(reinterpret_cast<const CT*>(d.aux) + (ptrdiff_t)min(lrow, d.mrem - 1) * d.ldx + min(lcol, d.xrem - 4));
#define AVAE_S_DMA(kt, buf)                                                                                             \
    { __builtin_amdgcn_global_load_lds((gp_t)(srcA + (size_t)(kt) * kTileBytesK), (lp_t)(smem + (buf) * kStage + wave * 1024), 16, 0, 0);          \
      __builtin_amdgcn_global_load_lds((gp_t)(srcB + (size_t)(kt) * kTileBytesK), (lp_t)(smem + (buf) * kStage + (4 + wave) * 1024), 16, 0, 0); }
    AVAE_STAMP(1)
    const int npro = nk < RING - 1 ? nk : RING - 1;
    for (int p = 0; p < npro; ++p) AVAE_S_DMA(p, p)
    const unsigned warmed = desc_warm(warm_lines, warm_n, wave);
    const int sw0 = (fq ^ (fr >> 1)) * 16;
    const int aoff = (wr * 16 + fr) * kTileBytesK, boff = (32 + wc * 16 + fr) * kTileBytesK;
    f32x4 acc = {0.f, 0.f, 0.f, 0.f};
    int buf = 0;
    for (int kt = 0; kt < nk; ++kt) {
        const int rem = nk - 1 - kt;
        if (rem >= 2) asm volatile("s_waitcnt vmcnt(4)" ::: "memory");
        else if (rem == 1) asm volatile("s_waitcnt vmcnt(2)" ::: "memory");
        else asm volatile("s_waitcnt vmcnt(0)" ::: "memory");
        asm volatile("s_barrier" ::: "memory");
        if (kt == 0) { AVAE_STAMP(2) }
        const unsigned char* Sb = smem + buf * kStage;
        const u32x4 a0 = *reinterpret_cast<const u32x4*>(Sb + aoff + sw0), b0 = *reinterpret_cast<const u32x4*>(Sb + boff + sw0);
        const int fill = buf == 0 ? RING - 1 : buf - 1;
        if (kt + RING - 1 < nk) AVAE_S_DMA(kt + RING - 1, fill)
        const u32x4 a1 = *reinterpret_cast<const u32x4*>(Sb + aoff + (sw0 ^ 64)), b1 = *reinterpret_cast<const u32x4*>(Sb + boff + (sw0 ^ 64));
        mma<CT>(b0, a0, acc);
        mma<CT>(b1, a1, acc);
        buf = buf + 1 == RING ? 0 : buf + 1;
    }
#undef AVAE_S_DMA
    AVAE_STAMP(3)
    if (lrow < d.mrem && lcol < d.nrem) {
        float v[4];
#pragma unroll
        for (int e = 0; e < 4; ++e) {
            if constexpr (KIND == 0) v[e] = act_fwd_t<ACT>(acc[e]);
            else v[e] = acc[e] * act_bwd_t<ACT>(quad_elem<CT>(yq, e));
        }
        store_row<CT>(reinterpret_cast<CT*>(d.out) + (size_t)lrow * d.ld0 + lcol, v, d.nrem - lcol);
    }
    asm volatile("" :: "s"(warmed));
    AVAE_STAMP(4)
    AVAE_STAMP_FLUSH()
}

thread_local LaunchEvents t_launch_events = {nullptr, nullptr};

#define AVAE_LAUNCH(kernel, grid, block, lds, stream, ...)                                                   \
    do {                                                                                                     \
        if (t_launch_events.start) {                                                                         \
            hipExtLaunchKernelGGL(kernel, grid, block, lds, stream, t_launch_events.start, t_launch_events.stop, 0, __VA_ARGS__); \
            t_launch_events = LaunchEvents{nullptr, nullptr};                                                \
        } else {                                                                                             \
            hipLaunchKernelGGL(kernel, grid, block, lds, stream, __VA_ARGS__);                               \
        }                                                                                                    \
    } while (0)

template <typename K> static void set_max_lds(K kernel) {
    (void)hipFuncSetAttribute(reinterpret_cast<const void*>(kernel), hipFuncAttributeMaxDynamicSharedMemorySize, 160 * 1024);
}

template <typename CT, bool MASK>
__global__ void __launch_bounds__(kThreads) k_small_loss(const LaunchArgs args, unsigned long long* stamps, int launch_id) {
    constexpr int BM = 32, RING = 4, ES = (int)sizeof(CT);
    constexpr int kStage = 64 * kTileBytesK;
    unsigned char* smem = avae_dyn_smem;
    float* red = reinterpret_cast<float*>(smem + RING * kStage);
#ifdef AVAE_STAMPS
    unsigned long long sv[kStampWords] = {0, 0, 0, 0, 0, 0, 0, 0};
#endif
    AVAE_STAMP(0)
    const int part = blockIdx.x & 7, idx = blockIdx.x >> 3;
    const WorkItem w = args.items[blockIdx.y];
    asm volatile("" :: "s"(w.A), "s"(w.B), "s"(w.out0), "s"(w.aux0), "s"(w.lda), "s"(w.ldb), "s"(w.K), "s"(w.ld0), "s"(w.ldx));
    int t;
    {
        const int nt = w.tiles_m * w.tiles_n;
        const int q = nt >> 3, r = nt & 7;
        if (idx >= q + (part < r ? 1 : 0)) return;
        t = (part < r ? part * (q + 1) : r * (q + 1) + (part - r) * q) + idx;
    }
    if (w.kind == K_LATENT) {
        latent_item<4, MASK>(w, t, red);
        AVAE_STAMP(4)
        AVAE_STAMP_FLUSH()
        return;
    }
    const int tid = threadIdx.x, lane = tid & 63, wave = __builtin_amdgcn_readfirstlane(tid >> 6);
    const int wr = wave >> 1, wc = wave & 1, fr = lane & 15, fq = lane >> 4;
    const int tm = t / w.tiles_n, tn = t - tm * w.tiles_n;
    const int m0 = tm * BM, n0 = tn * 32;
    const int nk = (w.K * ES) / kTileBytesK;
    typedef const __attribute__((address_space(1))) void* gp_t;
    typedef __attribute__((address_space(3))) void* lp_t;
    const int prow = wave * 8 + (lane >> 3), lc = ((lane & 7) ^ ((prow >> 1) & 7)) * 16;
    const unsigned char* srcA = reinterpret_cast<const unsigned char*>(w.A) + (size_t)(m0 + prow) * w.lda * ES + lc;
    const unsigned char* srcB = reinterpret_cast<const unsigned char*>(w.B) + (size_t)(n0 + prow) * w.ldb * ES + lc;
    const int orow = m0 + wr * 16 + fr, ocol = n0 + wc * 16 + 4 * fq;
    const f32x4 xq = *reinterpret_cast<const f32x4*>(reinterpret_cast<const float*>(w.aux0) + (size_t)min(orow, w.M - 1) * w.ldx + min(ocol, w.ldx - 4));
    const bool rpres = !MASK || w.present[(size_t)min(orow, w.M - 1) * w.present_ld] != 0;
#define AVAE_S_DMA(kt, buf)                                                                                             \
    { __builtin_amdgcn_global_load_lds((gp_t)(srcA + (size_t)(kt) * kTileBytesK), (lp_t)(smem + (buf) * kStage + wave * 1024), 16, 0, 0);          \
      __builtin_amdgcn_global_load_lds((gp_t)(srcB + (size_t)(kt) * kTileBytesK), (lp_t)(smem + (buf) * kStage + (4 + wave) * 1024), 16, 0, 0); }
    AVAE_STAMP(1)
    const int npro = nk < RING - 1 ? nk : RING - 1;
    for (int p = 0; p < npro; ++p) AVAE_S_DMA(p, p)
    const int sw0 = (fq ^ (fr >> 1)) * 16;
    const int aoff = (wr * 16 + fr) * kTileBytesK, boff = (32 + wc * 16 + fr) * kTileBytesK;
    f32x4 acc = {0.f, 0.f, 0.f, 0.f};
    int buf = 0;
    for (int kt = 0; kt < nk; ++kt) {
        const int rem = nk - 1 - kt;
        if (rem >= 2) asm volatile("s_waitcnt vmcnt(4)" ::: "memory");
        else if (rem == 1) asm volatile("s_waitcnt vmcnt(2)" ::: "memory");
        else asm volatile("s_waitcnt vmcnt(0)" ::: "memory");
        asm volatile("s_barrier" ::: "memory");
        if (kt == 0) { AVAE_STAMP(2) }
        const unsigned char* Sb = smem + buf * kStage;
        const u32x4 a0 = *reinterpret_cast<const u32x4*>(Sb + aoff + sw0), b0 = *reinterpret_cast<const u32x4*>(Sb + boff + sw0);
        const int fill = buf == 0 ? RING - 1 : buf - 1;
        if (kt + RING - 1 < nk) AVAE_S_DMA(kt + RING - 1, fill)
        const u32x4 a1 = *reinterpret_cast<const u32x4*>(Sb + aoff + (sw0 ^ 64)), b1 = *reinterpret_cast<const u32x4*>(Sb + boff + (sw0 ^ 64));
        mma<CT>(b0, a0, acc);
        mma<CT>(b1, a1, acc);
        buf = buf + 1 == RING ? 0 : buf + 1;
    }
#undef AVAE_S_DMA
    AVAE_STAMP(3)
    const float sc = w.scale;
    float csum = 0.0f, v[4];
#pragma unroll
    for (int e = 0; e < 4; ++e) {
        const bool ok = orow < w.M && ocol + e < w.N && rpres;
        float sl, da;
        if (w.binary) loss_bernoulli(acc[e], xq[e], sc, sl, da);
        else loss_gauss(acc[e], xq[e], sc, sl, da);
        csum += ok ? sl : 0.0f;
        v[e] = ok ? da : 0.0f;
    }
    if (orow < w.M && ocol < w.N) store_row<CT>(reinterpret_cast<CT*>(w.out0) + (size_t)orow * w.ld0 + ocol, v, w.N - ocol);
    const float total = block_sum<4>(csum, red);
    if (tid == 0) w.partial[w.slot_base + t] = total;
    AVAE_STAMP(4)
    AVAE_STAMP_FLUSH()
}
void launch_small_loss(int compute_dtype, const LaunchArgs& args, int grid_x, int grid_y, int lds_bytes, hipStream_t s, unsigned long long* stamps, int launch_id) {
    const dim3 grid(grid_x, grid_y), block(kThreads);
    bool masked = false;
    for (int i = 0; i < args.n_items; ++i) masked = masked || args.items[i].present != nullptr;
    if (masked) {
        if (compute_dtype == AVAE_BF16) AVAE_LAUNCH((k_small_loss<__bf16, true>), grid, block, lds_bytes, s, args, stamps, launch_id);
        else AVAE_LAUNCH((k_small_loss<float, true>), grid, block, lds_bytes, s, args, stamps, launch_id);
    } else if (compute_dtype == AVAE_BF16) AVAE_LAUNCH((k_small_loss<__bf16, false>), grid, block, lds_bytes, s, args, stamps, launch_id);
    else AVAE_LAUNCH((k_small_loss<float, false>), grid, block, lds_bytes, s, args, stamps, launch_id);
}

constexpr int kHeadStage = (32 + 64) * kTileBytesK, kHeadImg = 2 * 32 * kTileBytesK;
int small_head_lds_bytes() { return 4 * kHeadStage + kHeadImg + 64; }

template <typename CT> __device__ __forceinline__ void img_put(unsigned char* img, int row, int d, float v) {
    const int b = d * (int)sizeof(CT), bo = b & 127;
    *reinterpret_cast<CT*>(img + (b >> 7) * (32 * kTileBytesK) + row * kTileBytesK + ((((bo >> 4) ^ ((row >> 1) & 7)) << 4) | (bo & 15))) = to_ct<CT>(v);
}

template <typename CT, int ACT>
__global__ void __launch_bounds__(kThreads) k_small_latb(const LaunchArgs args, DevState* st, unsigned long long* stamps, int launch_id) {
    constexpr int RING = 4, ES = (int)sizeof(CT), TSL = ES == 2 ? 2 : 4;
    unsigned char* smem = avae_dyn_smem;
    unsigned char* img = smem + RING * kHeadStage;
    float* red = reinterpret_cast<float*>(img + kHeadImg);
#ifdef AVAE_STAMPS
    unsigned long long sv[kStampWords] = {0, 0, 0, 0, 0, 0, 0, 0};
#endif
    AVAE_STAMP(0)
    const int part = blockIdx.x & 7, idx = blockIdx.x >> 3;
    const WorkItem w = args.items[blockIdx.y];
    asm volatile("" :: "s"(w.A), "s"(w.B), "s"(w.out0), "s"(w.aux2), "s"(w.lda), "s"(w.ldb), "s"(w.K), "s"(w.ld0), "s"(w.tail_w), "s"(w.tail_out), "s"(w.tail_aux));
    int t;
    {
        const int nt = w.tiles_m * w.tiles_n;
        const int q = nt >> 3, r = nt & 7;
        if (idx >= q + (part < r ? 1 : 0)) return;
        t = (part < r ? part * (q + 1) : r * (q + 1) + (part - r) * q) + idx;
    }
    if (w.kind == K_COST) {
        cost_item<4>(w, st, red);
        AVAE_STAMP(4)
        AVAE_STAMP_FLUSH()
        return;
    }
    const int tid = threadIdx.x, lane = tid & 63, wave = __builtin_amdgcn_readfirstlane(tid >> 6);
    const int wr = wave >> 1, wc = wave & 1, fr = lane & 15, fq = lane >> 4;
    const int tm = t / w.tiles_n, ts = t - tm * w.tiles_n;
    const int m0 = tm * 32;
    const int nk = (w.K * ES) / kTileBytesK, nz = w.nz;
    typedef const __attribute__((address_space(1))) void* gp_t;
    typedef __attribute__((address_space(3))) void* lp_t;
    reinterpret_cast<f32x4*>(img)[tid] = f32x4{0.f, 0.f, 0.f, 0.f};
    reinterpret_cast<f32x4*>(img)[tid + kThreads] = f32x4{0.f, 0.f, 0.f, 0.f};
    const int orow = m0 + wr * 16 + fr;
    const int lde = (nz + 3) & ~3;
    const int t_i = wave & 1, t_c0 = (2 * ts + (wave >> 1)) * 32, t_sl = 2 * w.tail_kt;
    const int prow = wave * 8 + (lane >> 3), lc = ((lane & 7) ^ ((prow >> 1) & 7)) * 16;
    const unsigned char* srcA = reinterpret_cast<const unsigned char*>(w.A) + (size_t)(m0 + prow) * w.lda * ES + lc;
    const unsigned char* srcB = reinterpret_cast<const unsigned char*>(w.B) + (size_t)prow * w.ldb * ES + lc;
    const size_t b32 = (size_t)32 * w.ldb * ES;
#define AVAE_H_DMA(kt, buf)                                                                                             \
    { __builtin_amdgcn_global_load_lds((gp_t)(srcA + (size_t)(kt) * kTileBytesK), (lp_t)(smem + (buf) * kHeadStage + wave * 1024), 16, 0, 0);       \
      __builtin_amdgcn_global_load_lds((gp_t)(srcB + (size_t)(kt) * kTileBytesK), (lp_t)(smem + (buf) * kHeadStage + (4 + wave) * 1024), 16, 0, 0); \
      __builtin_amdgcn_global_load_lds((gp_t)(srcB + b32 + (size_t)(kt) * kTileBytesK), (lp_t)(smem + (buf) * kHeadStage + (8 + wave) * 1024), 16, 0, 0); }
    AVAE_STAMP(1)
    const int npro = nk < RING - 1 ? nk : RING - 1;
    for (int p = 0; p < npro; ++p) AVAE_H_DMA(p, p)
    constexpr int kExtra = 6 + 2 * TSL + 2;
    asm volatile("" ::: "memory"); __builtin_amdgcn_sched_barrier(0);
    f32x4 gm[2], gl[2], gf[2];
#pragma unroll
    for (int j = 0; j < 2; ++j) {
        const float* gr = reinterpret_cast<const float*>(w.aux2) + (size_t)min(orow, w.M - 1) * 3 * lde + min(wc * 32 + j * 16 + 4 * fq, lde - 4);
        gm[j] = *reinterpret_cast<const f32x4*>(gr); gl[j] = *reinterpret_cast<const f32x4*>(gr + lde); gf[j] = *reinterpret_cast<const f32x4*>(gr + 2 * lde);
    }
    u32x4 tb[TSL][2];
    typename Quad<CT>::raw ty[2];
#pragma unroll
    for (int j = 0; j < 2; ++j) {
        const unsigned char* pw = reinterpret_cast<const unsigned char*>(w.tail_w) + (size_t)min(t_c0 + 16 * j + fr, w.tail_n - 1) * w.tail_ldw * ES + fq * 16;
#pragma unroll
        for (int sl = 0; sl < TSL; ++sl) tb[sl][j] = *reinterpret_cast<const u32x4*>(pw + (sl < t_sl ? 64 * sl : 0));
        ty[j] = *reinterpret_cast<const typename Quad<CT>::raw*>(reinterpret_cast<const CT*>(w.tail_aux) + (size_t)min(m0 + 16 * t_i + fr, w.M - 1) * w.tail_ldx
                                                                   + min(t_c0 + 16 * j + 4 * fq, w.tail_ldx - 4));
    }
    asm volatile("" ::: "memory"); __builtin_amdgcn_sched_barrier(0);
    const int sw0 = (fq ^ (fr >> 1)) * 16;
    const int aoff = (wr * 16 + fr) * kTileBytesK, boff = (32 + wc * 32 + fr) * kTileBytesK;
    f32x4 acc[2] = {{0.f, 0.f, 0.f, 0.f}, {0.f, 0.f, 0.f, 0.f}};
    int buf = 0;
    for (int kt = 0; kt < nk; ++kt) {
        const int rem = nk - 1 - kt;
        if (kt < npro) {
            if (rem >= 2) asm volatile("s_waitcnt vmcnt(%0)" :: "n"(6 + kExtra) : "memory");
            else if (rem == 1) asm volatile("s_waitcnt vmcnt(%0)" :: "n"(3 + kExtra) : "memory");
            else asm volatile("s_waitcnt vmcnt(%0)" :: "n"(kExtra) : "memory");
        } else {
            if (rem >= 2) asm volatile("s_waitcnt vmcnt(6)" ::: "memory");
            else if (rem == 1) asm volatile("s_waitcnt vmcnt(3)" ::: "memory");
            else asm volatile("s_waitcnt vmcnt(0)" ::: "memory");
        }
        asm volatile("s_barrier" ::: "memory");
        if (kt == 0) { AVAE_STAMP(2) }
        const unsigned char* Sb = smem + buf * kHeadStage;
        const u32x4 a0 = *reinterpret_cast<const u32x4*>(Sb + aoff + sw0);
        const u32x4 b00 = *reinterpret_cast<const u32x4*>(Sb + boff + sw0), b01 = *reinterpret_cast<const u32x4*>(Sb + boff + 16 * kTileBytesK + sw0);
        const int fill = buf == 0 ? RING - 1 : buf - 1;
        if (kt + RING - 1 < nk) AVAE_H_DMA(kt + RING - 1, fill)
        const u32x4 a1 = *reinterpret_cast<const u32x4*>(Sb + aoff + (sw0 ^ 64));
        const u32x4 b10 = *reinterpret_cast<const u32x4*>(Sb + boff + (sw0 ^ 64)), b11 = *reinterpret_cast<const u32x4*>(Sb + boff + 16 * kTileBytesK + (sw0 ^ 64));
        mma<CT>(b00, a0, acc[0]); mma<CT>(b01, a0, acc[1]);
        mma<CT>(b10, a1, acc[0]); mma<CT>(b11, a1, acc[1]);
        buf = buf + 1 == RING ? 0 : buf + 1;
    }
#undef AVAE_H_DMA
    asm volatile("" :: "v"(ty[0]), "v"(ty[1]));
    AVAE_STAMP(3)
    {
        CT* dH = reinterpret_cast<CT*>(w.out0) + (size_t)orow * w.ld0;
        const bool store = ts == 0 && orow < w.M;
        const int lrow = wr * 16 + fr;
#pragma unroll
        for (int j = 0; j < 2; ++j)
#pragma unroll
            for (int e = 0; e < 4; ++e) {
                const int d = wc * 32 + j * 16 + 4 * fq + e;
                if (d < nz) {
                    const float dz = acc[j][e];
                    const float dmu = dz + gm[j][e], dlv = __builtin_fmaf(dz, gf[j][e], gl[j][e]);
                    img_put<CT>(img, lrow, d, dmu);
                    img_put<CT>(img, lrow, nz + d, dlv);
                    if (store) { dH[d] = to_ct<CT>(dmu); dH[nz + d] = to_ct<CT>(dlv); }
                }
            }
    }
    lds_barrier();
    AVAE_STAMP(5)
    {
        const int arow = 16 * t_i + fr;
        f32x4 tacc[1][2] = {{{0.f, 0.f, 0.f, 0.f}, {0.f, 0.f, 0.f, 0.f}}};
#pragma unroll
        for (int sl = 0; sl < TSL; ++sl)
            if (TSL == 2 || sl < t_sl) {
                const u32x4 ta = *reinterpret_cast<const u32x4*>(img + (sl >> 1) * (32 * kTileBytesK) + arow * kTileBytesK + (((fq + 4 * (sl & 1)) ^ ((arow >> 1) & 7)) << 4));
                mma<CT>(tb[sl][0], ta, tacc[0][0]);
                mma<CT>(tb[sl][1], ta, tacc[0][1]);
            }
        regep_store<CT, 1, 2>(tacc, reinterpret_cast<CT*>(w.tail_out), w.tail_ldo, w.M, w.tail_n, m0 + arow, t_c0, lane,
            [&](int, int j, int r, float v) { return v * act_bwd_t<ACT>(quad_elem<CT>(ty[j], r)); });
    }
    AVAE_STAMP(4)
    AVAE_STAMP_FLUSH()
}
template <typename CT, int ACT>
__global__ void __launch_bounds__(kThreads) k_small_head(const LaunchArgs args, unsigned long long* stamps, int launch_id) {
    constexpr int RING = 4, ES = (int)sizeof(CT), TSL = ES == 2 ? 2 : 4, LDM = 68;
    unsigned char* smem = avae_dyn_smem;
    unsigned char* img = smem + RING * kHeadStage;
    float* MV = reinterpret_cast<float*>(smem);
#ifdef AVAE_STAMPS
    unsigned long long sv[kStampWords] = {0, 0, 0, 0, 0, 0, 0, 0};
#endif
    AVAE_STAMP(0)
    const int part = blockIdx.x & 7, idx = blockIdx.x >> 3;
    const WorkItem w = args.items[blockIdx.y];
    asm volatile("" :: "s"(w.A), "s"(w.B), "s"(w.out0), "s"(w.out1), "s"(w.aux0), "s"(w.lda), "s"(w.ldb), "s"(w.K), "s"(w.ld0), "s"(w.tail_w), "s"(w.tail_out));
    int t;
    {
        const int nt = w.tiles_m * w.tiles_n;
        const int q = nt >> 3, r = nt & 7;
        if (idx >= q + (part < r ? 1 : 0)) return;
        t = (part < r ? part * (q + 1) : r * (q + 1) + (part - r) * q) + idx;
    }
    const int tid = threadIdx.x, lane = tid & 63, wave = __builtin_amdgcn_readfirstlane(tid >> 6);
    const int wr = wave >> 1, wc = wave & 1, fr = lane & 15, fq = lane >> 4;
    const int tm = t / w.tiles_n, ts = t - tm * w.tiles_n;
    const int m0 = tm * 32;
    const int nk = (w.K * ES) / kTileBytesK, nz = w.nz;
    typedef const __attribute__((address_space(1))) void* gp_t;
    typedef __attribute__((address_space(3))) void* lp_t;
    reinterpret_cast<f32x4*>(img)[tid] = f32x4{0.f, 0.f, 0.f, 0.f};
    reinterpret_cast<f32x4*>(img)[tid + kThreads] = f32x4{0.f, 0.f, 0.f, 0.f};
    const int zrow = tid >> 3, zg = tid & 7;
    const f32x4 ev = *reinterpret_cast<const f32x4*>(reinterpret_cast<const float*>(w.aux0) + (size_t)min(m0 + zrow, w.M - 1) * w.ldx + min(4 * zg, w.ldx - 4));
    const int t_i = wave & 1, t_c0 = (2 * ts + (wave >> 1)) * 32, t_sl = 2 * w.tail_kt;
    u32x4 tb[TSL][2];
#pragma unroll
    for (int j = 0; j < 2; ++j) {
        const unsigned char* pw = reinterpret_cast<const unsigned char*>(w.tail_w) + (size_t)min(t_c0 + 16 * j + fr, w.tail_n - 1) * w.tail_ldw * ES + fq * 16;
#pragma unroll
        for (int sl = 0; sl < TSL; ++sl) if (TSL == 2 || sl < t_sl) tb[sl][j] = *reinterpret_cast<const u32x4*>(pw + 64 * sl);
    }
    const int prow = wave * 8 + (lane >> 3), lc = ((lane & 7) ^ ((prow >> 1) & 7)) * 16;
    const unsigned char* srcA = reinterpret_cast<const unsigned char*>(w.A) + (size_t)(m0 + prow) * w.lda * ES + lc;
    const unsigned char* srcB = reinterpret_cast<const unsigned char*>(w.B) + (size_t)prow * w.ldb * ES + lc;
    const size_t b32 = (size_t)32 * w.ldb * ES;
#define AVAE_H_DMA(kt, buf)                                                                                             \
    { __builtin_amdgcn_global_load_lds((gp_t)(srcA + (size_t)(kt) * kTileBytesK), (lp_t)(smem + (buf) * kHeadStage + wave * 1024), 16, 0, 0);       \
      __builtin_amdgcn_global_load_lds((gp_t)(srcB + (size_t)(kt) * kTileBytesK), (lp_t)(smem + (buf) * kHeadStage + (4 + wave) * 1024), 16, 0, 0); \
      __builtin_amdgcn_global_load_lds((gp_t)(srcB + b32 + (size_t)(kt) * kTileBytesK), (lp_t)(smem + (buf) * kHeadStage + (8 + wave) * 1024), 16, 0, 0); }
    AVAE_STAMP(1)
    const int npro = nk < RING - 1 ? nk : RING - 1;
    for (int p = 0; p < npro; ++p) AVAE_H_DMA(p, p)
    const int sw0 = (fq ^ (fr >> 1)) * 16;
    const int aoff = (wr * 16 + fr) * kTileBytesK, boff = (32 + wc * 32 + fr) * kTileBytesK;
    f32x4 acc[2] = {{0.f, 0.f, 0.f, 0.f}, {0.f, 0.f, 0.f, 0.f}};
    int buf = 0;
    for (int kt = 0; kt < nk; ++kt) {
        const int rem = nk - 1 - kt;
        if (rem >= 2) asm volatile("s_waitcnt vmcnt(6)" ::: "memory");
        else if (rem == 1) asm volatile("s_waitcnt vmcnt(3)" ::: "memory");
        else asm volatile("s_waitcnt vmcnt(0)" ::: "memory");
        asm volatile("s_barrier" ::: "memory");
        if (kt == 0) { AVAE_STAMP(2) }
        const unsigned char* Sb = smem + buf * kHeadStage;
        const u32x4 a0 = *reinterpret_cast<const u32x4*>(Sb + aoff + sw0);
        const u32x4 b00 = *reinterpret_cast<const u32x4*>(Sb + boff + sw0), b01 = *reinterpret_cast<const u32x4*>(Sb + boff + 16 * kTileBytesK + sw0);
        const int fill = buf == 0 ? RING - 1 : buf - 1;
        if (kt + RING - 1 < nk) AVAE_H_DMA(kt + RING - 1, fill)
        const u32x4 a1 = *reinterpret_cast<const u32x4*>(Sb + aoff + (sw0 ^ 64));
        const u32x4 b10 = *reinterpret_cast<const u32x4*>(Sb + boff + (sw0 ^ 64)), b11 = *reinterpret_cast<const u32x4*>(Sb + boff + 16 * kTileBytesK + (sw0 ^ 64));
        mma<CT>(b00, a0, acc[0]); mma<CT>(b01, a0, acc[1]);
        mma<CT>(b10, a1, acc[0]); mma<CT>(b11, a1, acc[1]);
        buf = buf + 1 == RING ? 0 : buf + 1;
    }
#undef AVAE_H_DMA
    lds_barrier();
    AVAE_STAMP(3)
    {
        const int orow = m0 + wr * 16 + fr, lrow = wr * 16 + fr;
        float* mulv = reinterpret_cast<float*>(w.out0) + (size_t)orow * w.ld0;
        const bool store = ts == 0 && orow < w.M;
#pragma unroll
        for (int j = 0; j < 2; ++j) {
            const int c0 = wc * 32 + j * 16 + 4 * fq;
            *reinterpret_cast<f32x4*>(MV + lrow * LDM + c0) = acc[j];
            if (store) {
#pragma unroll
                for (int e = 0; e < 4; ++e) if (c0 + e < 2 * nz) mulv[c0 + e] = acc[j][e];
            }
        }
    }
    lds_barrier();
    AVAE_STAMP(5)
    {
        CT* Z = reinterpret_cast<CT*>(w.out1) + (size_t)(m0 + zrow) * w.ld1;
        const bool store = ts == 0 && m0 + zrow < w.M;
#pragma unroll
        for (int e = 0; e < 4; ++e) {
            const int d = 4 * zg + e;
            if (d < nz) {
                const float z = __builtin_fmaf(fexp(0.5f * MV[zrow * LDM + nz + d]), ev[e], MV[zrow * LDM + d]);
                img_put<CT>(img, zrow, d, z);
                if (store) Z[d] = to_ct<CT>(z);
            }
        }
        if (tid < 32) img_put<CT>(img, tid, nz, 1.0f);
    }
    lds_barrier();
    AVAE_STAMP_EP(6)
    {
        const int arow = 16 * t_i + fr;
        f32x4 tacc[1][2] = {{{0.f, 0.f, 0.f, 0.f}, {0.f, 0.f, 0.f, 0.f}}};
#pragma unroll
        for (int sl = 0; sl < TSL; ++sl)
            if (TSL == 2 || sl < t_sl) {
                const u32x4 ta = *reinterpret_cast<const u32x4*>(img + (sl >> 1) * (32 * kTileBytesK) + arow * kTileBytesK + (((fq + 4 * (sl & 1)) ^ ((arow >> 1) & 7)) << 4));
                mma<CT>(tb[sl][0], ta, tacc[0][0]);
                mma<CT>(tb[sl][1], ta, tacc[0][1]);
            }
        regep_store<CT, 1, 2>(tacc, reinterpret_cast<CT*>(w.tail_out), w.tail_ldo, w.M, w.tail_n, m0 + arow, t_c0, lane,
            [&](int, int, int, float v) { return act_fwd_t<ACT>(v); });
    }
    AVAE_STAMP(4)
    AVAE_STAMP_FLUSH()
}
void launch_small_head(int compute_dtype, int act, const LaunchArgs& args, int grid_x, int grid_y, int lds_bytes, hipStream_t s,
                       unsigned long long* stamps, int launch_id) {
    const dim3 grid(grid_x, grid_y), block(kThreads);
#define K_HEAD_B(A) k_small_head<__bf16, A>
#define K_HEAD_F(A) k_small_head<float, A>
    if (compute_dtype == AVAE_BF16) {
        switch (act) {
            case AVAE_ACT_RELU: AVAE_LAUNCH((K_HEAD_B(AVAE_ACT_RELU)), grid, block, lds_bytes, s, args, stamps, launch_id); break;
            case AVAE_ACT_SOFTPLUS: AVAE_LAUNCH((K_HEAD_B(AVAE_ACT_SOFTPLUS)), grid, block, lds_bytes, s, args, stamps, launch_id); break;
            case AVAE_ACT_SIGMOID: AVAE_LAUNCH((K_HEAD_B(AVAE_ACT_SIGMOID)), grid, block, lds_bytes, s, args, stamps, launch_id); break;
            case AVAE_ACT_TANH: AVAE_LAUNCH((K_HEAD_B(AVAE_ACT_TANH)), grid, block, lds_bytes, s, args, stamps, launch_id); break;
            default: AVAE_LAUNCH((K_HEAD_B(AVAE_ACT_IDENTITY)), grid, block, lds_bytes, s, args, stamps, launch_id); break;
        }
    } else {
        switch (act) {
            case AVAE_ACT_RELU: AVAE_LAUNCH((K_HEAD_F(AVAE_ACT_RELU)), grid, block, lds_bytes, s, args, stamps, launch_id); break;
            case AVAE_ACT_SOFTPLUS: AVAE_LAUNCH((K_HEAD_F(AVAE_ACT_SOFTPLUS)), grid, block, lds_bytes, s, args, stamps, launch_id); break;
            case AVAE_ACT_SIGMOID: AVAE_LAUNCH((K_HEAD_F(AVAE_ACT_SIGMOID)), grid, block, lds_bytes, s, args, stamps, launch_id); break;
            case AVAE_ACT_TANH: AVAE_LAUNCH((K_HEAD_F(AVAE_ACT_TANH)), grid, block, lds_bytes, s, args, stamps, launch_id); break;
            default: AVAE_LAUNCH((K_HEAD_F(AVAE_ACT_IDENTITY)), grid, block, lds_bytes, s, args, stamps, launch_id); break;
        }
    }
#undef K_HEAD_B
#undef K_HEAD_F
}
void launch_small_latb(int compute_dtype, int act, const LaunchArgs& args, int grid_x, int grid_y, int lds_bytes, DevState* st, hipStream_t s,
                       unsigned long long* stamps, int launch_id) {
    const dim3 grid(grid_x, grid_y), block(kThreads);
#define K_LATB_B(A) k_small_latb<__bf16, A>
#define K_LATB_F(A) k_small_latb<float, A>
    if (compute_dtype == AVAE_BF16) {
        switch (act) {
            case AVAE_ACT_RELU: AVAE_LAUNCH((K_LATB_B(AVAE_ACT_RELU)), grid, block, lds_bytes, s, args, st, stamps, launch_id); break;
            case AVAE_ACT_SOFTPLUS: AVAE_LAUNCH((K_LATB_B(AVAE_ACT_SOFTPLUS)), grid, block, lds_bytes, s, args, st, stamps, launch_id); break;
            case AVAE_ACT_SIGMOID: AVAE_LAUNCH((K_LATB_B(AVAE_ACT_SIGMOID)), grid, block, lds_bytes, s, args, st, stamps, launch_id); break;
            case AVAE_ACT_TANH: AVAE_LAUNCH((K_LATB_B(AVAE_ACT_TANH)), grid, block, lds_bytes, s, args, st, stamps, launch_id); break;
            default: AVAE_LAUNCH((K_LATB_B(AVAE_ACT_IDENTITY)), grid, block, lds_bytes, s, args, st, stamps, launch_id); break;
        }
    } else {
        switch (act) {
            case AVAE_ACT_RELU: AVAE_LAUNCH((K_LATB_F(AVAE_ACT_RELU)), grid, block, lds_bytes, s, args, st, stamps, launch_id); break;
            case AVAE_ACT_SOFTPLUS: AVAE_LAUNCH((K_LATB_F(AVAE_ACT_SOFTPLUS)), grid, block, lds_bytes, s, args, st, stamps, launch_id); break;
            case AVAE_ACT_SIGMOID: AVAE_LAUNCH((K_LATB_F(AVAE_ACT_SIGMOID)), grid, block, lds_bytes, s, args, st, stamps, launch_id); break;
            case AVAE_ACT_TANH: AVAE_LAUNCH((K_LATB_F(AVAE_ACT_TANH)), grid, block, lds_bytes, s, args, st, stamps, launch_id); break;
            default: AVAE_LAUNCH((K_LATB_F(AVAE_ACT_IDENTITY)), grid, block, lds_bytes, s, args, st, stamps, launch_id); break;
        }
    }
#undef K_LATB_B
#undef K_LATB_F
}

#ifdef AVAE_STAMPS
#define AVAE_SV sv
#else
#define AVAE_SV nullptr
#endif
template <typename CT, bool ADAM, typename F>
__device__ __forceinline__ void small_tn_tile(const TnDesc& d, const TnDescArgs& ca, F&& behind_prologue, unsigned char* smem, unsigned long long* sv) {
    constexpr int BM = 64, RING = 4, ES = (int)sizeof(CT), EPR = kTileBytesK / ES, NCH = 4;
    constexpr int kStage = 2 * BM * kTileBytesK;
    const int tid = threadIdx.x, lane = tid & 63, wave = __builtin_amdgcn_readfirstlane(tid >> 6);
    const int wr = wave >> 1, wc = wave & 1, fr = lane & 15, fq = lane >> 4;
    const int nk = d.ext & 0xFFFF, mrem = (d.ext >> 16) & 0xFF, nrem = d.ext >> 24;
    typedef const __attribute__((address_space(1))) void* gp_t;
    typedef __attribute__((address_space(3))) void* lp_t;
    const unsigned char* src[NCH];
    size_t kadv[NCH];
#pragma unroll
    for (int c = 0; c < NCH; ++c) {
        const int r = (c * 4 + wave) * 8 + (lane >> 3);
        const bool is_a = c < 2;
        const int rr = is_a ? r : r - BM, sub = rr / EPR, k = rr - sub * EPR;
        const int lc = (lane & 7) ^ tn_swz<CT>(k);
        const size_t ld_b = (size_t)(is_a ? d.lda : d.ldb) * ES;
        kadv[c] = (size_t)EPR * ld_b;
        src[c] = (is_a ? d.a : d.b) + (size_t)k * ld_b + (size_t)sub * kTileBytesK + lc * 16;
    }
#define AVAE_T_DMA(kt, buf)                                                                                             \
    { _Pragma("unroll") for (int c = 0; c < NCH; ++c)                                                                   \
        __builtin_amdgcn_global_load_lds((gp_t)(src[c] + (size_t)(kt) * kadv[c]), (lp_t)(smem + (buf) * kStage + (c * 4 + wave) * 1024), 16, 0, 0); }
    int offA[2], offB[2];
#pragma unroll
    for (int i = 0; i < 2; ++i) { offA[i] = tn_frag_off<CT>(wr * 32 + i * 16, lane); offB[i] = BM * kTileBytesK + tn_frag_off<CT>(wc * 32 + i * 16, lane); }
    AVAE_STAMP(1)
    const int npro = nk < RING - 1 ? nk : RING - 1;
    for (int p = 0; p < npro; ++p) AVAE_T_DMA(p, p)
    const float lr_t = behind_prologue();
    const int c4 = (tid & 15) * 4;
    f32x4 pth[4], pmm[4], pvv[4];
    auto fetch_state = [&]() {
#pragma unroll
        for (int k = 0; k < 4; ++k) {
            const int lrow = (tid >> 4) + 16 * k;
            const bool ok = lrow < mrem && c4 < nrem;
            const float* gp = d.out + (size_t)(ok ? lrow : 0) * d.ld0 + (ok ? c4 : 0);
            pth[k] = *reinterpret_cast<const f32x4*>(gp + ca.d_theta);
            pmm[k] = *reinterpret_cast<const f32x4*>(gp + ca.d_m);
            pvv[k] = *reinterpret_cast<const f32x4*>(gp + ca.d_v);
        }
    };
    f32x4 acc[2][2];
#pragma unroll
    for (int i = 0; i < 2; ++i)
#pragma unroll
        for (int j = 0; j < 2; ++j) acc[i][j] = f32x4{0.f, 0.f, 0.f, 0.f};
    int buf = 0;
    for (int kt = 0; kt < nk; ++kt) {
        const int rem = nk - 1 - kt;
        if (rem >= 2) asm volatile("s_waitcnt vmcnt(8)" ::: "memory");
        else if (rem == 1) asm volatile("s_waitcnt vmcnt(4)" ::: "memory");
        else asm volatile("s_waitcnt vmcnt(0)" ::: "memory");
        asm volatile("s_barrier" ::: "memory");
        if (kt == 0) { AVAE_STAMP(2) }
        const unsigned char* Sb = smem + buf * kStage;
        u32x4 a0[2], b0[2], a1[2], b1[2];
#pragma unroll
        for (int i = 0; i < 2; ++i) { a0[i] = tn_frag<CT>(Sb, offA[i], 0); b0[i] = tn_frag<CT>(Sb, offB[i], 0); }
        const int fill = buf == 0 ? RING - 1 : buf - 1;
        if (kt + RING - 1 < nk) AVAE_T_DMA(kt + RING - 1, fill)
#pragma unroll
        for (int i = 0; i < 2; ++i) { a1[i] = tn_frag<CT>(Sb, offA[i], 1); b1[i] = tn_frag<CT>(Sb, offB[i], 1); }
        if constexpr (sizeof(CT) == 2) { tn_wait_lds(); tn_frags_ready(a0); tn_frags_ready(b0); tn_frags_ready(a1); tn_frags_ready(b1); }
#pragma unroll
        for (int i = 0; i < 2; ++i)
#pragma unroll
            for (int j = 0; j < 2; ++j) mma<CT>(b0[j], a0[i], acc[i][j]);
#pragma unroll
        for (int i = 0; i < 2; ++i)
#pragma unroll
            for (int j = 0; j < 2; ++j) mma<CT>(b1[j], a1[i], acc[i][j]);
        buf = buf + 1 == RING ? 0 : buf + 1;
    }
#undef AVAE_T_DMA
    AVAE_STAMP(3)
    if constexpr (!ADAM) {
#pragma unroll
        for (int i = 0; i < 2; ++i) {
            const int row = wr * 32 + i * 16 + fr;
#pragma unroll
            for (int j = 0; j < 2; ++j) {
                const int col = wc * 32 + j * 16 + 4 * fq;
                if (row < mrem && col < nrem) {
                    const float g[4] = {acc[i][j][0], acc[i][j][1], acc[i][j][2], acc[i][j][3]};
                    store_row<float>(d.out + (size_t)row * d.ld0 + col, g, nrem - col);
                }
            }
        }
    } else {
        constexpr int LDT = 65;
        float* T = reinterpret_cast<float*>(smem);
        fetch_state();
        lds_barrier();
#pragma unroll
        for (int i = 0; i < 2; ++i)
#pragma unroll
            for (int j = 0; j < 2; ++j)
#pragma unroll
                for (int e = 0; e < 4; ++e) T[(wr * 32 + i * 16 + fr) * LDT + wc * 32 + j * 16 + 4 * fq + e] = acc[i][j][e];
        lds_barrier();
        const float omb1 = 1.0f - ca.beta1, omb2 = 1.0f - ca.beta2;
        const int r4 = (tid & 15) * 4;
        float g[4][4], th[4][4], m[4][4], v[4][4];
#pragma unroll
        for (int k = 0; k < 4; ++k) {
            const int r = (tid >> 4) + 16 * k;
#pragma unroll
            for (int e = 0; e < 4; ++e) { g[k][e] = T[r * LDT + c4 + e]; th[k][e] = pth[k][e]; m[k][e] = pmm[k][e]; v[k][e] = pvv[k][e]; }
#pragma unroll
            for (int e = 0; e < 4; ++e) adam_update(g[k][e], m[k][e], v[k][e], th[k][e], omb1, omb2, lr_t, ca.eps);
#pragma unroll
            for (int e = 0; e < 4; ++e) T[r * LDT + c4 + e] = th[k][e];
        }
        const bool full = mrem >= BM && nrem >= BM;
        auto store_group = [&](int k, float* gp, CT* wp) {
            store4<float>(gp, g[k]);
            store4<float>(gp + ca.d_theta, th[k]); store4<float>(gp + ca.d_m, m[k]); store4<float>(gp + ca.d_v, v[k]);
            store4<CT>(wp, th[k]);
        };
        if (full) {
#pragma unroll
            for (int k = 0; k < 4; ++k) {
                const int lrow = (tid >> 4) + 16 * k;
                store_group(k, d.out + (size_t)lrow * d.ld0 + c4, reinterpret_cast<CT*>(d.w) + (size_t)lrow * d.ldw + c4);
            }
        } else {
#pragma unroll
            for (int k = 0; k < 4; ++k) {
                const int lrow = (tid >> 4) + 16 * k;
                float* gp = d.out + (size_t)lrow * d.ld0 + c4;
                CT* wp = reinterpret_cast<CT*>(d.w) + (size_t)lrow * d.ldw + c4;
                const int nv = nrem - c4;
                if (lrow < mrem && nv >= 4) {
                    store_group(k, gp, wp);
                } else if (lrow < mrem && nv > 0) {
#pragma unroll
                    for (int e = 0; e < 3; ++e) if (e < nv) {
                        gp[e] = g[k][e]; gp[ca.d_theta + e] = th[k][e]; gp[ca.d_m + e] = m[k][e]; gp[ca.d_v + e] = v[k][e]; wp[e] = to_ct<CT>(th[k][e]);
                    }
                    asm volatile("; partial quad" ::: "memory");
                }
            }
        }
        lds_barrier();
#pragma unroll
        for (int k = 0; k < 4; ++k) {
            const int cc = (tid >> 4) + 16 * k;
            float t[4];
#pragma unroll
            for (int e = 0; e < 4; ++e) t[e] = T[(r4 + e) * LDT + cc];
// ... 1962 lines not shown
```

Baseline: 4.987 million.

## Drive loss, head and latent-backward kernels from precomputed per-tile records

Extends the descriptor-table scheme to the loss (cfg 9), forward head (cfg 11) and latent-backward (cfg 10) launches. The host precomputes a 128-byte record per tile holding base pointers, strides and remainders, dealt across XCDs. Each block reads its record instead of decoding WorkItems and tile indices, and warms the next launch's records behind its DMA prologue. This is meant to cut per-block setup latency in these small, latency-bound kernels. It adds table memory, warm-line logic for paired lines, and separate paths for the masked and non-plain variants, which strip the records.

```diff
diff --git a/vae_assoc_amd/csrc/avae_device.h b/vae_assoc_amd/csrc/avae_device.h
--- a/vae_assoc_amd/csrc/avae_device.h
+++ b/vae_assoc_amd/csrc/avae_device.h
@@ -163,6 +163,42 @@
     static constexpr unsigned pack(int nk, int mrem, int nrem) { return (unsigned)nk | (unsigned)(mrem < 64 ? mrem : 64) << 16 | (unsigned)(nrem < 64 ? nrem : 64) << 24; }
 };
 static_assert(sizeof(SmallDesc) == 64 && sizeof(TnDesc) == 64, "a descriptor is one cache line");
+struct alignas(128) LossRec {
+    const unsigned char* a;
+    const unsigned char* b;
+    void* out;
+    const float* x;
+    float* slot;
+    int lda, ldb, ld0, ldx;
+    int nk;
+    int mrem, nrem, xrem;
+    float scale;
+    int binary;
+    int item, tile;
+    int pad_[10];
+};
+struct alignas(128) HeadRec {
+    const unsigned char* a;
+    const unsigned char* b;
+    void* out0;
+    void* out1;
+    const float* aux;
+    const unsigned char* tail_w;
+    void* tail_out;
+    const void* tail_aux;
+    int lda, ldb, ld0, ld1, ldx;
+    int tail_ldw, tail_ldo, tail_ldx;
+    int nk, nz;
+    int mrem;
+    int tail_n;
+    unsigned tk;
+    int item;
+    int pad_[2];
+    static constexpr unsigned pack(int tail_kt, int ts) { return (unsigned)tail_kt | (unsigned)ts << 8; }
+};
+static_assert(sizeof(LossRec) == 128 && sizeof(HeadRec) == 128, "a head or loss record is two cache lines");
+static_assert(sizeof(LaunchArgs) + 64 <= 4096, "the record kernels pass LaunchArgs by value behind their leading arguments: 4 KiB");
+constexpr int kWarmPairs = 1 << 30;
 struct DescWarm { const void* lines; int n; };
 struct TnDescArgs {
     long long d_theta, d_m, d_v;
@@ -502,6 +538,12 @@
 void launch_small_desc(int compute_dtype, bool dgrad, int act, const SmallDesc* tab, int n_tiles, int lds_bytes, DescWarm warm, hipStream_t s,
                        unsigned long long* stamps, int launch_id);
 void launch_small_tn_desc(int compute_dtype, const TnDesc* tab, int n_tiles, DescWarm warm, hipStream_t s, unsigned long long* stamps, int launch_id);
+void launch_loss_rec(int compute_dtype, const LossRec* tab, int n_recs, int lds_bytes, DescWarm warm, const LaunchArgs& args, hipStream_t s,
+                     unsigned long long* stamps, int launch_id);
+void launch_head_rec(int compute_dtype, int act, const HeadRec* tab, int n_recs, int lds_bytes, DescWarm warm, hipStream_t s,
+                     unsigned long long* stamps, int launch_id);
+void launch_latb_rec(int compute_dtype, int act, const HeadRec* tab, int n_recs, int lds_bytes, DescWarm warm, DevState* st, const LaunchArgs& args,
+                     hipStream_t s, unsigned long long* stamps, int launch_id);
 void launch_reduce(const ReduceArgs& a, int n_blocks, hipStream_t s);
 void launch_chain2(int compute_dtype, const LaunchArgs& args, int grid_x, int grid_y, int lds_bytes, unsigned* counters, unsigned* err, hipStream_t s);
 
diff --git a/vae_assoc_amd/csrc/avae_host.hip b/vae_assoc_amd/csrc/avae_host.hip
--- a/vae_assoc_amd/csrc/avae_host.hip
+++ b/vae_assoc_amd/csrc/avae_host.hip
@@ -1991,18 +1991,104 @@
     return deal_to_xcds(lists);
 }
 
+template <typename F> void tiles_of_part(const WorkItem& w, int part, F&& f) {
+    const int nt = w.tiles_m * w.tiles_n, q = nt >> 3, r = nt & 7;
+    for (int idx = 0; idx < q + (part < r ? 1 : 0); ++idx) f((part < r ? part * (q + 1) : r * (q + 1) + (part - r) * q) + idx);
+}
+
+std::vector<LossRec> loss_recs(const avae_handle* h, const Launch& L) {
+    std::vector<LossRec> lists[8];
+    const int es = h->es;
+    for (int y = 0; y < L.args.n_items; ++y) {
+        const WorkItem& w = L.args.items[y];
+        if ((w.kind != K_FWD_OUT_LOSS && w.kind != K_LATENT) || w.present || w.conv > 0 || w.bias_ep) return {};
+        for (int part = 0; part < 8; ++part)
+            tiles_of_part(w, part, [&](int t) {
+                LossRec d{};
+                d.item = -1;
+                if (w.kind == K_LATENT) { d.item = y; d.tile = t; lists[part].push_back(d); return; }
+                const int tm = t / w.tiles_n, tn = t - tm * w.tiles_n, m0 = tm * 32, n0 = tn * 32;
+                d.a = static_cast<const unsigned char*>(w.A) + (size_t)m0 * w.lda * es;
+                d.b = static_cast<const unsigned char*>(w.B) + (size_t)n0 * w.ldb * es;
+                d.out = static_cast<unsigned char*>(w.out0) + ((size_t)m0 * w.ld0 + n0) * es;
+                d.x = static_cast<const float*>(w.aux0) + (size_t)m0 * w.ldx + n0;
+                d.slot = w.partial + w.slot_base + t;
+                d.lda = w.lda; d.ldb = w.ldb; d.ld0 = w.ld0; d.ldx = w.ldx;
+                d.nk = (w.K * es) / kTileBytesK;
+                d.mrem = w.M - m0; d.nrem = w.N - n0; d.xrem = w.ldx - n0;
+                d.scale = w.scale; d.binary = w.binary;
+                lists[part].push_back(d);
+            });
+    }
+    return deal_to_xcds(lists);
+}
+
+std::vector<HeadRec> head_recs(const avae_handle* h, const Launch& L) {
+    std::vector<HeadRec> lists[8];
+    const int es = h->es;
+    const bool bwd = L.cfg == 10;
+    for (int y = 0; y < L.args.n_items; ++y) {
+        const WorkItem& w = L.args.items[y];
+        const bool cost = bwd && w.kind == K_COST;
+        if (!cost && (w.kind != (bwd ? K_DGRAD_LATENT : K_FWD_HEAD) || w.tail_mode != (bwd ? 2 : 1) || w.tail_act != L.lean_act)) return {};
+        if (!cost && (w.present || w.conv > 0 || w.bias_ep || w.tail_kt < 1 || w.tail_kt > 2)) return {};
+        for (int part = 0; part < 8; ++part)
+            tiles_of_part(w, part, [&](int t) {
+                HeadRec d{};
+                d.item = -1;
+                if (cost) { d.item = y; lists[part].push_back(d); return; }
+                const int tm = t / w.tiles_n, ts = t - tm * w.tiles_n, m0 = tm * 32;
+                d.a = static_cast<const unsigned char*>(w.A) + (size_t)m0 * w.lda * es;
+                d.b = static_cast<const unsigned char*>(w.B);
+                d.tail_w = static_cast<const unsigned char*>(w.tail_w);
+                d.tail_out = static_cast<unsigned char*>(w.tail_out) + (size_t)m0 * w.tail_ldo * es;
+                if (bwd) {
+                    d.out0 = static_cast<unsigned char*>(w.out0) + (size_t)m0 * w.ld0 * es;
+                    d.aux = static_cast<const float*>(w.aux2) + (size_t)m0 * 3 * ((w.nz + 3) & ~3);
+                    d.tail_aux = static_cast<const unsigned char*>(w.tail_aux) + (size_t)m0 * w.tail_ldx * es;
+                } else {
+                    d.out0 = static_cast<float*>(w.out0) + (size_t)m0 * w.ld0;
+                    d.out1 = static_cast<unsigned char*>(w.out1) + (size_t)m0 * w.ld1 * es;
+                    d.aux = static_cast<const float*>(w.aux0) + (size_t)m0 * w.ldx;
+                }
+                d.lda = w.lda; d.ldb = w.ldb; d.ld0 = w.ld0; d.ld1 = w.ld1; d.ldx = w.ldx;
+                d.tail_ldw = w.tail_ldw; d.tail_ldo = w.tail_ldo; d.tail_ldx = w.tail_ldx;
+                d.nk = (w.K * es) / kTileBytesK; d.nz = w.nz;
+                d.mrem = w.M - m0; d.tail_n = w.tail_n;
+                d.tk = HeadRec::pack(w.tail_kt, ts);
+                lists[part].push_back(d);
+            });
+    }
+    return deal_to_xcds(lists);
+}
+
+bool two_line_records(const Launch& L) { return L.type == 0 && !L.tn && (L.cfg == 9 || L.cfg == 10 || L.cfg == 11); }
+
 void build_descriptors(avae_handle* h, hipStream_t s) {
     if (std::getenv("AVAE_NO_DESC")) return;
     std::vector<unsigned char> tab;
     auto add = [&](Launch& L) {
-        if (L.type != 0 || !((L.cfg == 7 && !L.tn) || (L.cfg == 12 && L.tn && L.targs.adam))) return;
+        if (L.type != 0 || !((L.cfg == 7 && !L.tn) || (L.cfg == 12 && L.tn && L.targs.adam) || two_line_records(L))) return;
+        tab.resize((tab.size() + 127) & ~(size_t)127);
         const size_t off = tab.size();
         size_t stride = 0;
         int n = 0;
+        auto put = [&](const auto& d) {
+            if (d.empty()) { tab.resize(off); return false; }
+            const size_t at = tab.size(), bytes = d.size() * sizeof(d[0]);
+            tab.resize(at + bytes);
+            std::memcpy(tab.data() + at, d.data(), bytes);
+            n = (int)d.size();
+            return true;
+        };
         for (int j = 0; j < kMultiSteps; ++j) {
             const Launch Lj = j == 0 ? L : relocated(h, L, j);
             const size_t at = tab.size();
-            if (L.tn) {
+            if (L.cfg == 9) {
+                if (!put(loss_recs(h, Lj))) return;
+            } else if (L.cfg == 10 || L.cfg == 11) {
+                if (!put(head_recs(h, Lj))) return;
+            } else if (L.tn) {
                 const std::vector<TnDesc> d = tn_descs(h, Lj);
                 if (d.empty()) { tab.resize(off); return; }
                 const TnDescArgs ca = {L.targs.d_theta, L.targs.d_m, L.targs.d_v, L.targs.beta1, L.targs.beta2, L.targs.eps, L.targs.st};
@@ -2035,13 +2121,13 @@
 
 DescWarm warm_for(const avae_handle* h, const Launch* next, int next_set) {
     if (!next || next->desc_n == 0 || next_set >= kMultiSteps) return DescWarm{nullptr, 0};
-    return DescWarm{h->desc_buf.as<unsigned char>() + next->desc_off + (size_t)next_set * next->desc_stride,
-                    next->desc_n + (next->tn ? kTnDescHead : 0)};
+    const int lines = two_line_records(*next) ? 2 * next->desc_n | kWarmPairs : next->desc_n + (next->tn ? kTnDescHead : 0);
+    return DescWarm{h->desc_buf.as<unsigned char>() + next->desc_off + (size_t)next_set * next->desc_stride, lines};
 }
 
 void dump_launch(const Launch& L) {
     std::fprintf(stderr, "[avae] launch %s type=%d cfg=%d items=%d blocks=%d\n", L.name.c_str(), L.type, L.cfg, L.count, L.blocks);
-    if (L.desc_n) std::fprintf(stderr, "        descriptors=%d set=%d\n", L.desc_n, L.desc_set);
+    if (L.desc_n) std::fprintf(stderr, two_line_records(L) ? "        records=%d set=%d\n" : "        descriptors=%d set=%d\n", L.desc_n, L.desc_set);
     for (int i = 0; i < L.args.n_items && L.type == 0; ++i)
         std::fprintf(stderr, "        item kind=%d M=%d N=%d K=%d lda=%d ldb=%d tiles=%dx%d\n", L.args.items[i].kind, L.args.items[i].M,
                      L.args.items[i].N, L.args.items[i].K, L.args.items[i].lda, L.args.items[i].ldb, L.args.items[i].tiles_m, L.args.items[i].tiles_n);
@@ -2066,6 +2152,9 @@
     else if (L.type == 8) launch_rowsum(h->cfg.compute_dtype, L.rs, L.blocks, s);
     else if (L.type == 9) launch_sums(L.ra, L.blocks, s);
     else if (L.cfg == 13) launch_chain2(h->cfg.compute_dtype, L.args, L.grid_x, L.grid_y, L.lds, h->at<unsigned>(h->off_chain), h->at<unsigned>(h->off_chain) + kMaxMod * 64, s);
+    else if (L.cfg == 11 && L.desc_n) launch_head_rec(h->cfg.compute_dtype, L.lean_act, desc_of<HeadRec>(h, L), L.desc_n, L.lds, warm, s, stamps, stamp);
+    else if (L.cfg == 10 && L.desc_n) launch_latb_rec(h->cfg.compute_dtype, L.lean_act, desc_of<HeadRec>(h, L), L.desc_n, L.lds, warm, h->state(), L.args, s, stamps, stamp);
+    else if (L.cfg == 9 && L.desc_n) launch_loss_rec(h->cfg.compute_dtype, desc_of<LossRec>(h, L), L.desc_n, L.lds, warm, L.args, s, stamps, stamp);
     else if (L.cfg == 11) launch_small_head(h->cfg.compute_dtype, L.lean_act, L.args, L.grid_x, L.grid_y, L.lds, s, stamps, stamp);
     else if (L.cfg == 10) launch_small_latb(h->cfg.compute_dtype, L.lean_act, L.args, L.grid_x, L.grid_y, L.lds, h->state(), s, stamps, stamp);
     else if (L.cfg == 9) launch_small_loss(h->cfg.compute_dtype, L.args, L.grid_x, L.grid_y, L.lds, s, stamps, stamp);
@@ -2090,7 +2179,7 @@
 }
 
 void run_set(avae_handle* h, const std::vector<Launch>& ls, size_t lo, size_t hi, int j, hipStream_t s, int stamp_base = -1, bool train = false,
-             const Launch* after = nullptr, int after_set = 0) {
+             const Launch* after = nullptr, int after_set = 0, bool records2 = true) {
     unsigned long long* stamps = nullptr;
 #ifdef AVAE_STAMPS
     if (stamp_base >= 0) stamps = h->at<unsigned long long>(h->off_stamps);
@@ -2105,8 +2194,11 @@
         const int k = stamp_base + (int)(i - lo);
         const bool last = i + 1 >= hi || i + 1 >= ls.size();
         const DescWarm warm = last ? warm_for(h, after, after_set) : warm_for(h, &ls[i + 1], j);
-        if (j == 0 && !(hyper && has_hyper_item(ls[i]))) run_launch(h, ls[i], s, stamps, k, warm);
-        else run_launch(h, relocated(h, ls[i], j, hyper), s, stamps, k, warm);
+        const bool strip = !records2 && ls[i].desc_n && two_line_records(ls[i]);
+        if (j == 0 && !(hyper && has_hyper_item(ls[i])) && !strip) { run_launch(h, ls[i], s, stamps, k, warm); continue; }
+        Launch L = relocated(h, ls[i], j, hyper);
+        if (strip) L.desc_n = 0;
+        run_launch(h, L, s, stamps, k, warm);
     }
 }
 
@@ -2278,7 +2370,8 @@
     auto first_of = [](const std::vector<Launch>& ls) { return ls.empty() ? nullptr : &ls[0]; };
     const bool fused = !h->wgrad_adam.empty() && !h->clip_on && !h->ema_on;
     run_set(h, fwd, 0, fwd.size(), j, s, stamp_base, true, first_of(h->bwd), j);
-    run_set(h, h->bwd, 0, h->bwd.size(), j, s, sb(fwd.size()), true, fused ? first_of(h->wgrad_adam) : nullptr, j);
+    const bool plain = &fwd == &h->plain.fwd;
+    run_set(h, h->bwd, 0, h->bwd.size(), j, s, sb(fwd.size()), true, fused ? first_of(h->wgrad_adam) : nullptr, j, plain);
     if (fused) {
         run_set(h, h->wgrad_adam, 0, h->wgrad_adam.size(), j, s, sb(fwd.size() + h->bwd.size()), true, more ? first_of(fwd) : nullptr, j + 1);
         return;
@@ -2970,6 +3063,7 @@
     }
     if (n_loss != h->M || n_latent != 1) throw Err("internal error: the masked twin found " + std::to_string(n_loss) + " loss and " +
                                                    std::to_string(n_latent) + " latent items");
+    for (Launch& L : mf) if (two_line_records(L)) L.desc_n = 0;
     h->masked.fwd.swap(mf);
     if (h->cfg.use_graph) {
         try { capture_plan(h, h->masked, pres); } catch (...) { h->masked.fwd.clear(); throw; }
diff --git a/vae_assoc_amd/csrc/avae_kernels.hip b/vae_assoc_amd/csrc/avae_kernels.hip
--- a/vae_assoc_amd/csrc/avae_kernels.hip
+++ b/vae_assoc_amd/csrc/avae_kernels.hip
@@ -1301,7 +1301,8 @@
 __device__ __forceinline__ unsigned desc_warm(const void* lines, int n, int wave) {
     typedef const __attribute__((address_space(4))) unsigned* cu_t;
     const int i = (blockIdx.x & 7) + 8 * (4 * (blockIdx.x >> 3) + wave);
-    return i < n ? *(cu_t)((unsigned long long)lines + 64ull * (unsigned)i) : 0u;
+    const int line = (n & kWarmPairs) ? 2 * ((i & 7) + 8 * (i >> 4)) + ((i >> 3) & 1) : i;
+    return line < (n & ~kWarmPairs) ? *(cu_t)((unsigned long long)lines + 64ull * (unsigned)line) : 0u;
 }
 
 template <typename CT, int KIND, int ACT>
@@ -1386,6 +1387,76 @@
     (void)hipFuncSetAttribute(reinterpret_cast<const void*>(kernel), hipFuncAttributeMaxDynamicSharedMemorySize, 160 * 1024);
 }
 
+#ifdef AVAE_STAMPS
+#define AVAE_SV sv
+#else
+#define AVAE_SV nullptr
+#endif
+template <typename T> __device__ __forceinline__ T* as_global(T* p) {
+    return (T*)(__attribute__((address_space(1))) T*)(unsigned long long)p;
+}
+template <typename CT, bool MASK, typename F>
+__device__ __forceinline__ void small_loss_tile(const LossRec& d, const unsigned char* present, int present_ld, F&& behind_prologue,
+                                                unsigned char* smem, float* red, unsigned long long* sv) {
+    constexpr int RING = 4, ES = (int)sizeof(CT);
+    constexpr int kStage = 64 * kTileBytesK;
+    const int tid = threadIdx.x, lane = tid & 63, wave = __builtin_amdgcn_readfirstlane(tid >> 6);
+    const int wr = wave >> 1, wc = wave & 1, fr = lane & 15, fq = lane >> 4;
+    const int nk = d.nk;
+    typedef const __attribute__((address_space(1))) void* gp_t;
+    typedef __attribute__((address_space(3))) void* lp_t;
+    const int prow = wave * 8 + (lane >> 3), lc = ((lane & 7) ^ ((prow >> 1) & 7)) * 16;
+    const unsigned char* srcA = d.a + (size_t)prow * d.lda * ES + lc;
+    const unsigned char* srcB = d.b + (size_t)prow * d.ldb * ES + lc;
+    const int lrow = wr * 16 + fr, lcol = wc * 16 + 4 * fq;
+    const f32x4 xq = *reinterpret_cast<const f32x4*>(as_global(d.x) + (ptrdiff_t)min(lrow, d.mrem - 1) * d.ldx + min(lcol, d.xrem - 4));
+    bool rpres = true;
+    if constexpr (MASK) rpres = as_global(present)[(size_t)min(lrow, d.mrem - 1) * present_ld] != 0;
+#define AVAE_S_DMA(kt, buf)                                                                                             \
+    { __builtin_amdgcn_global_load_lds((gp_t)(srcA + (size_t)(kt) * kTileBytesK), (lp_t)(smem + (buf) * kStage + wave * 1024), 16, 0, 0);          \
+      __builtin_amdgcn_global_load_lds((gp_t)(srcB + (size_t)(kt) * kTileBytesK), (lp_t)(smem + (buf) * kStage + (4 + wave) * 1024), 16, 0, 0); }
+    AVAE_STAMP(1)
+    const int npro = nk < RING - 1 ? nk : RING - 1;
+    for (int p = 0; p < npro; ++p) AVAE_S_DMA(p, p)
+    behind_prologue();
+    const int sw0 = (fq ^ (fr >> 1)) * 16;
+    const int aoff = (wr * 16 + fr) * kTileBytesK, boff = (32 + wc * 16 + fr) * kTileBytesK;
+    f32x4 acc = {0.f, 0.f, 0.f, 0.f};
+    int buf = 0;
+    for (int kt = 0; kt < nk; ++kt) {
+        const int rem = nk - 1 - kt;
+        if (rem >= 2) asm volatile("s_waitcnt vmcnt(4)" ::: "memory");
+        else if (rem == 1) asm volatile("s_waitcnt vmcnt(2)" ::: "memory");
+        else asm volatile("s_waitcnt vmcnt(0)" ::: "memory");
+        asm volatile("s_barrier" ::: "memory");
+        if (kt == 0) { AVAE_STAMP(2) }
+        const unsigned char* Sb = smem + buf * kStage;
+        const u32x4 a0 = *reinterpret_cast<const u32x4*>(Sb + aoff + sw0), b0 = *reinterpret_cast<const u32x4*>(Sb + boff + sw0);
+        const int fill = buf == 0 ? RING - 1 : buf - 1;
+        if (kt + RING - 1 < nk) AVAE_S_DMA(kt + RING - 1, fill)
+        const u32x4 a1 = *reinterpret_cast<const u32x4*>(Sb + aoff + (sw0 ^ 64)), b1 = *reinterpret_cast<const u32x4*>(Sb + boff + (sw0 ^ 64));
+        mma<CT>(b0, a0, acc);
+        mma<CT>(b1, a1, acc);
+        buf = buf + 1 == RING ? 0 : buf + 1;
+    }
+#undef AVAE_S_DMA
+    AVAE_STAMP(3)
+    const float sc = d.scale;
+    float csum = 0.0f, v[4];
+#pragma unroll
+    for (int e = 0; e < 4; ++e) {
+        const bool ok = lrow < d.mrem && lcol + e < d.nrem && rpres;
+        float sl, da;
+        if (d.binary) loss_bernoulli(acc[e], xq[e], sc, sl, da);
+        else loss_gauss(acc[e], xq[e], sc, sl, da);
+        csum += ok ? sl : 0.0f;
+        v[e] = ok ? da : 0.0f;
+    }
+    if (lrow < d.mrem && lcol < d.nrem) store_row<CT>(as_global(reinterpret_cast<CT*>(d.out)) + (size_t)lrow * d.ld0 + lcol, v, d.nrem - lcol);
+    const float total = block_sum<4>(csum, red);
+    if (tid == 0) *as_global(d.slot) = total;
+}
+
 template <typename CT, bool MASK>
 __global__ void __launch_bounds__(kThreads) k_small_loss(const LaunchArgs args, unsigned long long* stamps, int launch_id) {
     constexpr int BM = 32, RING = 4, ES = (int)sizeof(CT);
@@ -1412,63 +1483,55 @@
         AVAE_STAMP_FLUSH()
         return;
     }
-    const int tid = threadIdx.x, lane = tid & 63, wave = __builtin_amdgcn_readfirstlane(tid >> 6);
-    const int wr = wave >> 1, wc = wave & 1, fr = lane & 15, fq = lane >> 4;
     const int tm = t / w.tiles_n, tn = t - tm * w.tiles_n;
     const int m0 = tm * BM, n0 = tn * 32;
-    const int nk = (w.K * ES) / kTileBytesK;
-    typedef const __attribute__((address_space(1))) void* gp_t;
-    typedef __attribute__((address_space(3))) void* lp_t;
-    const int prow = wave * 8 + (lane >> 3), lc = ((lane & 7) ^ ((prow >> 1) & 7)) * 16;
-    const unsigned char* srcA = reinterpret_cast<const unsigned char*>(w.A) + (size_t)(m0 + prow) * w.lda * ES + lc;
-    const unsigned char* srcB = reinterpret_cast<const unsigned char*>(w.B) + (size_t)(n0 + prow) * w.ldb * ES + lc;
-    const int orow = m0 + wr * 16 + fr, ocol = n0 + wc * 16 + 4 * fq;
-    const f32x4 xq = *reinterpret_cast<const f32x4*>(reinterpret_cast<const float*>(w.aux0) + (size_t)min(orow, w.M - 1) * w.ldx + min(ocol, w.ldx - 4));
-    const bool rpres = !MASK || w.present[(size_t)min(orow, w.M - 1) * w.present_ld] != 0;
-#define AVAE_S_DMA(kt, buf)                                                                                             \
-    { __builtin_amdgcn_global_load_lds((gp_t)(srcA + (size_t)(kt) * kTileBytesK), (lp_t)(smem + (buf) * kStage + wave * 1024), 16, 0, 0);          \
-      __builtin_amdgcn_global_load_lds((gp_t)(srcB + (size_t)(kt) * kTileBytesK), (lp_t)(smem + (buf) * kStage + (4 + wave) * 1024), 16, 0, 0); }
-    AVAE_STAMP(1)
-    const int npro = nk < RING - 1 ? nk : RING - 1;
-    for (int p = 0; p < npro; ++p) AVAE_S_DMA(p, p)
-    const int sw0 = (fq ^ (fr >> 1)) * 16;
-    const int aoff = (wr * 16 + fr) * kTileBytesK, boff = (32 + wc * 16 + fr) * kTileBytesK;
-    f32x4 acc = {0.f, 0.f, 0.f, 0.f};
-    int buf = 0;
-    for (int kt = 0; kt < nk; ++kt) {
-        const int rem = nk - 1 - kt;
-        if (rem >= 2) asm volatile("s_waitcnt vmcnt(4)" ::: "memory");
-        else if (rem == 1) asm volatile("s_waitcnt vmcnt(2)" ::: "memory");
-        else asm volatile("s_waitcnt vmcnt(0)" ::: "memory");
-        asm volatile("s_barrier" ::: "memory");
-        if (kt == 0) { AVAE_STAMP(2) }
-        const unsigned char* Sb = smem + buf * kStage;
-        const u32x4 a0 = *reinterpret_cast<const u32x4*>(Sb + aoff + sw0), b0 = *reinterpret_cast<const u32x4*>(Sb + boff + sw0);
-        const int fill = buf == 0 ? RING - 1 : buf - 1;
-        if (kt + RING - 1 < nk) AVAE_S_DMA(kt + RING - 1, fill)
-        const u32x4 a1 = *reinterpret_cast<const u32x4*>(Sb + aoff + (sw0 ^ 64)), b1 = *reinterpret_cast<const u32x4*>(Sb + boff + (sw0 ^ 64));
-        mma<CT>(b0, a0, acc);
-        mma<CT>(b1, a1, acc);
-        buf = buf + 1 == RING ? 0 : buf + 1;
-    }
-#undef AVAE_S_DMA
-    AVAE_STAMP(3)
-    const float sc = w.scale;
-    float csum = 0.0f, v[4];
-#pragma unroll
-    for (int e = 0; e < 4; ++e) {
-        const bool ok = orow < w.M && ocol + e < w.N && rpres;
-        float sl, da;
-        if (w.binary) loss_bernoulli(acc[e], xq[e], sc, sl, da);
-        else loss_gauss(acc[e], xq[e], sc, sl, da);
-        csum += ok ? sl : 0.0f;
-        v[e] = ok ? da : 0.0f;
-    }
-    if (orow < w.M && ocol < w.N) store_row<CT>(reinterpret_cast<CT*>(w.out0) + (size_t)orow * w.ld0 + ocol, v, w.N - ocol);
-    const float total = block_sum<4>(csum, red);
-    if (tid == 0) w.partial[w.slot_base + t] = total;
+    LossRec d;
+    d.a = reinterpret_cast<const unsigned char*>(w.A) + (size_t)m0 * w.lda * ES;
+    d.b = reinterpret_cast<const unsigned char*>(w.B) + (size_t)n0 * w.ldb * ES;
+    d.out = reinterpret_cast<CT*>(w.out0) + (size_t)m0 * w.ld0 + n0;
+    d.x = reinterpret_cast<const float*>(w.aux0) + (size_t)m0 * w.ldx + n0;
+    d.slot = w.partial + w.slot_base + t;
+    d.lda = w.lda; d.ldb = w.ldb; d.ld0 = w.ld0; d.ldx = w.ldx;
+    d.nk = (w.K * ES) / kTileBytesK;
+    d.mrem = w.M - m0; d.nrem = w.N - n0; d.xrem = w.ldx - n0;
+    d.scale = w.scale; d.binary = w.binary;
+    const unsigned char* present = nullptr;
+    if constexpr (MASK) present = w.present + (size_t)m0 * w.present_ld;
+    small_loss_tile<CT, MASK>(d, present, w.present_ld, []() {}, smem, red, AVAE_SV);
     AVAE_STAMP(4)
     AVAE_STAMP_FLUSH()
+}
+
+template <typename CT>
+__global__ void __launch_bounds__(kThreads) k_loss_rec(const LossRec* __restrict__ tab, unsigned long long* stamps, int launch_id,
+                                                       const void* warm_lines, int warm_n, const LaunchArgs args) {
+    unsigned char* smem = avae_dyn_smem;
+    float* red = reinterpret_cast<float*>(smem + 4 * 64 * kTileBytesK);
+#ifdef AVAE_STAMPS
+    unsigned long long sv[kStampWords] = {0, 0, 0, 0, 0, 0, 0, 0};
+#endif
+    AVAE_STAMP(0)
+    const LossRec d = tab[blockIdx.x];
+    asm volatile("" :: "s"(d.a), "s"(d.b), "s"(d.out), "s"(d.x), "s"(d.slot), "s"(d.lda), "s"(d.ldb), "s"(d.ld0), "s"(d.ldx), "s"(d.nk), "s"(d.mrem),
+                 "s"(d.nrem), "s"(d.xrem), "s"(d.scale), "s"(d.binary), "s"(d.item), "s"(d.tile));
+    if (d.item >= 0) {
+        latent_item<4, false>(args.items[d.item], d.tile, red);
+        AVAE_STAMP(4)
+        AVAE_STAMP_FLUSH()
+        return;
+    }
+    unsigned warmed = 0;
+    small_loss_tile<CT, false>(d, nullptr, 0, [&]() { warmed = desc_warm(warm_lines, warm_n, __builtin_amdgcn_readfirstlane(threadIdx.x >> 6)); },
+                               smem, red, AVAE_SV);
+    asm volatile("" :: "s"(warmed));
+    AVAE_STAMP(4)
+    AVAE_STAMP_FLUSH()
+}
+void launch_loss_rec(int compute_dtype, const LossRec* tab, int n_recs, int lds_bytes, DescWarm warm, const LaunchArgs& args, hipStream_t s,
+                     unsigned long long* stamps, int launch_id) {
+    const dim3 grid(n_recs), block(kThreads);
+    if (compute_dtype == AVAE_BF16) AVAE_LAUNCH((k_loss_rec<__bf16>), grid, block, lds_bytes, s, tab, stamps, launch_id, warm.lines, warm.n, args);
+    else AVAE_LAUNCH((k_loss_rec<float>), grid, block, lds_bytes, s, tab, stamps, launch_id, warm.lines, warm.n, args);
 }
 void launch_small_loss(int compute_dtype, const LaunchArgs& args, int grid_x, int grid_y, int lds_bytes, hipStream_t s, unsigned long long* stamps, int launch_id) {
     const dim3 grid(grid_x, grid_y), block(kThreads);
@@ -1489,48 +1552,25 @@
     *reinterpret_cast<CT*>(img + (b >> 7) * (32 * kTileBytesK) + row * kTileBytesK + ((((bo >> 4) ^ ((row >> 1) & 7)) << 4) | (bo & 15))) = to_ct<CT>(v);
 }
 
-template <typename CT, int ACT>
-__global__ void __launch_bounds__(kThreads) k_small_latb(const LaunchArgs args, DevState* st, unsigned long long* stamps, int launch_id) {
+template <typename CT, int ACT, typename F>
+__device__ __forceinline__ void small_latb_tile(const HeadRec& d, F&& behind_prologue, unsigned char* smem, unsigned long long* sv) {
     constexpr int RING = 4, ES = (int)sizeof(CT), TSL = ES == 2 ? 2 : 4;
-    unsigned char* smem = avae_dyn_smem;
     unsigned char* img = smem + RING * kHeadStage;
-    float* red = reinterpret_cast<float*>(img + kHeadImg);
-#ifdef AVAE_STAMPS
-    unsigned long long sv[kStampWords] = {0, 0, 0, 0, 0, 0, 0, 0};
-#endif
-    AVAE_STAMP(0)
-    const int part = blockIdx.x & 7, idx = blockIdx.x >> 3;
-    const WorkItem w = args.items[blockIdx.y];
-    asm volatile("" :: "s"(w.A), "s"(w.B), "s"(w.out0), "s"(w.aux2), "s"(w.lda), "s"(w.ldb), "s"(w.K), "s"(w.ld0), "s"(w.tail_w), "s"(w.tail_out), "s"(w.tail_aux));
-    int t;
-    {
-        const int nt = w.tiles_m * w.tiles_n;
-        const int q = nt >> 3, r = nt & 7;
-        if (idx >= q + (part < r ? 1 : 0)) return;
-        t = (part < r ? part * (q + 1) : r * (q + 1) + (part - r) * q) + idx;
-    }
-    if (w.kind == K_COST) {
-        cost_item<4>(w, st, red);
-        AVAE_STAMP(4)
-        AVAE_STAMP_FLUSH()
-        return;
-    }
     const int tid = threadIdx.x, lane = tid & 63, wave = __builtin_amdgcn_readfirstlane(tid >> 6);
     const int wr = wave >> 1, wc = wave & 1, fr = lane & 15, fq = lane >> 4;
-    const int tm = t / w.tiles_n, ts = t - tm * w.tiles_n;
-    const int m0 = tm * 32;
-    const int nk = (w.K * ES) / kTileBytesK, nz = w.nz;
+    const int ts = d.tk >> 8;
+    const int nk = d.nk, nz = d.nz;
     typedef const __attribute__((address_space(1))) void* gp_t;
     typedef __attribute__((address_space(3))) void* lp_t;
     reinterpret_cast<f32x4*>(img)[tid] = f32x4{0.f, 0.f, 0.f, 0.f};
     reinterpret_cast<f32x4*>(img)[tid + kThreads] = f32x4{0.f, 0.f, 0.f, 0.f};
-    const int orow = m0 + wr * 16 + fr;
+    const int lrow = wr * 16 + fr;
     const int lde = (nz + 3) & ~3;
-    const int t_i = wave & 1, t_c0 = (2 * ts + (wave >> 1)) * 32, t_sl = 2 * w.tail_kt;
+    const int t_i = wave & 1, t_c0 = (2 * ts + (wave >> 1)) * 32, t_sl = 2 * (int)(d.tk & 0xFF);
     const int prow = wave * 8 + (lane >> 3), lc = ((lane & 7) ^ ((prow >> 1) & 7)) * 16;
-    const unsigned char* srcA = reinterpret_cast<const unsigned char*>(w.A) + (size_t)(m0 + prow) * w.lda * ES + lc;
-    const unsigned char* srcB = reinterpret_cast<const unsigned char*>(w.B) + (size_t)prow * w.ldb * ES + lc;
-    const size_t b32 = (size_t)32 * w.ldb * ES;
+    const unsigned char* srcA = d.a + (size_t)prow * d.lda * ES + lc;
+    const unsigned char* srcB = d.b + (size_t)prow * d.ldb * ES + lc;
+    const size_t b32 = (size_t)32 * d.ldb * ES;
 #define AVAE_H_DMA(kt, buf)                                                                                             \
     { __builtin_amdgcn_global_load_lds((gp_t)(srcA + (size_t)(kt) * kTileBytesK), (lp_t)(smem + (buf) * kHeadStage + wave * 1024), 16, 0, 0);       \
       __builtin_amdgcn_global_load_lds((gp_t)(srcB + (size_t)(kt) * kTileBytesK), (lp_t)(smem + (buf) * kHeadStage + (4 + wave) * 1024), 16, 0, 0); \
@@ -1543,20 +1583,21 @@
     f32x4 gm[2], gl[2], gf[2];
 #pragma unroll
     for (int j = 0; j < 2; ++j) {
-        const float* gr = reinterpret_cast<const float*>(w.aux2) + (size_t)min(orow, w.M - 1) * 3 * lde + min(wc * 32 + j * 16 + 4 * fq, lde - 4);
+        const float* gr = as_global(d.aux) + (size_t)min(lrow, d.mrem - 1) * 3 * lde + min(wc * 32 + j * 16 + 4 * fq, lde - 4);
         gm[j] = *reinterpret_cast<const f32x4*>(gr); gl[j] = *reinterpret_cast<const f32x4*>(gr + lde); gf[j] = *reinterpret_cast<const f32x4*>(gr + 2 * lde);
     }
     u32x4 tb[TSL][2];
     typename Quad<CT>::raw ty[2];
 #pragma unroll
     for (int j = 0; j < 2; ++j) {
-        const unsigned char* pw = reinterpret_cast<const unsigned char*>(w.tail_w) + (size_t)min(t_c0 + 16 * j + fr, w.tail_n - 1) * w.tail_ldw * ES + fq * 16;
+        const unsigned char* pw = as_global(d.tail_w) + (size_t)min(t_c0 + 16 * j + fr, d.tail_n - 1) * d.tail_ldw * ES + fq * 16;
 #pragma unroll
         for (int sl = 0; sl < TSL; ++sl) tb[sl][j] = *reinterpret_cast<const u32x4*>(pw + (sl < t_sl ? 64 * sl : 0));
-        ty[j] = *reinterpret_cast<const typename Quad<CT>::raw*>(reinterpret_cast<const CT*>(w.tail_aux) + (size_t)min(m0 + 16 * t_i + fr, w.M - 1) * w.tail_ldx
-                                                                   + min(t_c0 + 16 * j + 4 * fq, w.tail_ldx - 4));
+        ty[j] = *reinterpret_cast<const typename Quad<CT>::raw*>(as_global(reinterpret_cast<const CT*>(d.tail_aux)) + (size_t)min(16 * t_i + fr, d.mrem - 1) * d.tail_ldx
+                                                                   + min(t_c0 + 16 * j + 4 * fq, d.tail_ldx - 4));
     }
     asm volatile("" ::: "memory"); __builtin_amdgcn_sched_barrier(0);
+    behind_prologue();
     const int sw0 = (fq ^ (fr >> 1)) * 16;
     const int aoff = (wr * 16 + fr) * kTileBytesK, boff = (32 + wc * 32 + fr) * kTileBytesK;
     f32x4 acc[2] = {{0.f, 0.f, 0.f, 0.f}, {0.f, 0.f, 0.f, 0.f}};
@@ -1589,20 +1630,19 @@
     asm volatile("" :: "v"(ty[0]), "v"(ty[1]));
     AVAE_STAMP(3)
     {
-        CT* dH = reinterpret_cast<CT*>(w.out0) + (size_t)orow * w.ld0;
-        const bool store = ts == 0 && orow < w.M;
-        const int lrow = wr * 16 + fr;
+        CT* dH = as_global(reinterpret_cast<CT*>(d.out0)) + (size_t)lrow * d.ld0;
+        const bool store = ts == 0 && lrow < d.mrem;
 #pragma unroll
         for (int j = 0; j < 2; ++j)
 #pragma unroll
             for (int e = 0; e < 4; ++e) {
-                const int d = wc * 32 + j * 16 + 4 * fq + e;
-                if (d < nz) {
+                const int dim = wc * 32 + j * 16 + 4 * fq + e;
+                if (dim < nz) {
                     const float dz = acc[j][e];
                     const float dmu = dz + gm[j][e], dlv = __builtin_fmaf(dz, gf[j][e], gl[j][e]);
-                    img_put<CT>(img, lrow, d, dmu);
-                    img_put<CT>(img, lrow, nz + d, dlv);
-                    if (store) { dH[d] = to_ct<CT>(dmu); dH[nz + d] = to_ct<CT>(dlv); }
+                    img_put<CT>(img, lrow, dim, dmu);
+                    img_put<CT>(img, lrow, nz + dim, dlv);
+                    if (store) { dH[dim] = to_ct<CT>(dmu); dH[nz + dim] = to_ct<CT>(dlv); }
                 }
             }
     }
@@ -1618,25 +1658,23 @@
                 mma<CT>(tb[sl][0], ta, tacc[0][0]);
                 mma<CT>(tb[sl][1], ta, tacc[0][1]);
             }
-        regep_store<CT, 1, 2>(tacc, reinterpret_cast<CT*>(w.tail_out), w.tail_ldo, w.M, w.tail_n, m0 + arow, t_c0, lane,
+        regep_store<CT, 1, 2>(tacc, as_global(reinterpret_cast<CT*>(d.tail_out)), d.tail_ldo, d.mrem, d.tail_n, arow, t_c0, lane,
             [&](int, int j, int r, float v) { return v * act_bwd_t<ACT>(quad_elem<CT>(ty[j], r)); });
     }
-    AVAE_STAMP(4)
-    AVAE_STAMP_FLUSH()
-}
+}
+
 template <typename CT, int ACT>
-__global__ void __launch_bounds__(kThreads) k_small_head(const LaunchArgs args, unsigned long long* stamps, int launch_id) {
-    constexpr int RING = 4, ES = (int)sizeof(CT), TSL = ES == 2 ? 2 : 4, LDM = 68;
+__global__ void __launch_bounds__(kThreads) k_small_latb(const LaunchArgs args, DevState* st, unsigned long long* stamps, int launch_id) {
+    constexpr int ES = (int)sizeof(CT);
     unsigned char* smem = avae_dyn_smem;
-    unsigned char* img = smem + RING * kHeadStage;
-    float* MV = reinterpret_cast<float*>(smem);
+    float* red = reinterpret_cast<float*>(smem + 4 * kHeadStage + kHeadImg);
 #ifdef AVAE_STAMPS
     unsigned long long sv[kStampWords] = {0, 0, 0, 0, 0, 0, 0, 0};
 #endif
     AVAE_STAMP(0)
     const int part = blockIdx.x & 7, idx = blockIdx.x >> 3;
     const WorkItem w = args.items[blockIdx.y];
-    asm volatile("" :: "s"(w.A), "s"(w.B), "s"(w.out0), "s"(w.out1), "s"(w.aux0), "s"(w.lda), "s"(w.ldb), "s"(w.K), "s"(w.ld0), "s"(w.tail_w), "s"(w.tail_out));
+    asm volatile("" :: "s"(w.A), "s"(w.B), "s"(w.out0), "s"(w.aux2), "s"(w.lda), "s"(w.ldb), "s"(w.K), "s"(w.ld0), "s"(w.tail_w), "s"(w.tail_out), "s"(w.tail_aux));
     int t;
     {
         const int nt = w.tiles_m * w.tiles_n;
@@ -1644,29 +1682,82 @@
         if (idx >= q + (part < r ? 1 : 0)) return;
         t = (part < r ? part * (q + 1) : r * (q + 1) + (part - r) * q) + idx;
     }
+    if (w.kind == K_COST) {
+        cost_item<4>(w, st, red);
+        AVAE_STAMP(4)
+        AVAE_STAMP_FLUSH()
+        return;
+    }
+    const int tm = t / w.tiles_n, ts = t - tm * w.tiles_n;
+    const int m0 = tm * 32;
+    HeadRec d;
+    d.a = reinterpret_cast<const unsigned char*>(w.A) + (size_t)m0 * w.lda * ES;
+    d.b = reinterpret_cast<const unsigned char*>(w.B);
+    d.out0 = reinterpret_cast<CT*>(w.out0) + (size_t)m0 * w.ld0;
+    d.aux = reinterpret_cast<const float*>(w.aux2) + (size_t)m0 * 3 * ((w.nz + 3) & ~3);
+    d.tail_w = reinterpret_cast<const unsigned char*>(w.tail_w);
+    d.tail_out = reinterpret_cast<CT*>(w.tail_out) + (size_t)m0 * w.tail_ldo;
+    d.tail_aux = reinterpret_cast<const CT*>(w.tail_aux) + (size_t)m0 * w.tail_ldx;
+    d.lda = w.lda; d.ldb = w.ldb; d.ld0 = w.ld0;
+    d.tail_ldw = w.tail_ldw; d.tail_ldo = w.tail_ldo; d.tail_ldx = w.tail_ldx;
+    d.nk = (w.K * ES) / kTileBytesK; d.nz = w.nz;
+    d.mrem = w.M - m0; d.tail_n = w.tail_n;
+    d.tk = HeadRec::pack(w.tail_kt, ts);
+    small_latb_tile<CT, ACT>(d, []() {}, smem, AVAE_SV);
+    AVAE_STAMP(4)
+    AVAE_STAMP_FLUSH()
+}
+
+template <typename CT, int ACT>
+__global__ void __launch_bounds__(kThreads) k_latb_rec(const HeadRec* __restrict__ tab, unsigned long long* stamps, int launch_id,
+                                                       const void* warm_lines, int warm_n, DevState* st, const LaunchArgs args) {
+    unsigned char* smem = avae_dyn_smem;
+#ifdef AVAE_STAMPS
+    unsigned long long sv[kStampWords] = {0, 0, 0, 0, 0, 0, 0, 0};
+#endif
+    AVAE_STAMP(0)
+    const HeadRec d = tab[blockIdx.x];
+    asm volatile("" :: "s"(d.a), "s"(d.b), "s"(d.out0), "s"(d.aux), "s"(d.tail_w), "s"(d.tail_out), "s"(d.tail_aux), "s"(d.lda), "s"(d.ldb), "s"(d.ld0),
+                 "s"(d.tail_ldw), "s"(d.tail_ldo), "s"(d.tail_ldx), "s"(d.nk), "s"(d.nz), "s"(d.mrem), "s"(d.tail_n), "s"(d.tk), "s"(d.item));
+    if (d.item >= 0) {
+        cost_item<4>(args.items[d.item], st, reinterpret_cast<float*>(smem + 4 * kHeadStage + kHeadImg));
+        AVAE_STAMP(4)
+        AVAE_STAMP_FLUSH()
+        return;
+    }
+    unsigned warmed = 0;
+    small_latb_tile<CT, ACT>(d, [&]() { warmed = desc_warm(warm_lines, warm_n, __builtin_amdgcn_readfirstlane(threadIdx.x >> 6)); }, smem, AVAE_SV);
+    asm volatile("" :: "s"(warmed));
+    AVAE_STAMP(4)
+    AVAE_STAMP_FLUSH()
+}
+template <typename CT, int ACT, typename F>
+__device__ __forceinline__ void small_head_tile(const HeadRec& d, F&& behind_prologue, unsigned char* smem, unsigned long long* sv) {
+    constexpr int RING = 4, ES = (int)sizeof(CT), TSL = ES == 2 ? 2 : 4, LDM = 68;
+    unsigned char* img = smem + RING * kHeadStage;
+    float* MV = reinterpret_cast<float*>(smem);
     const int tid = threadIdx.x, lane = tid & 63, wave = __builtin_amdgcn_readfirstlane(tid >> 6);
     const int wr = wave >> 1, wc = wave & 1, fr = lane & 15, fq = lane >> 4;
-    const int tm = t / w.tiles_n, ts = t - tm * w.tiles_n;
-    const int m0 = tm * 32;
-    const int nk = (w.K * ES) / kTileBytesK, nz = w.nz;
+    const int ts = d.tk >> 8;
+    const int nk = d.nk, nz = d.nz;
     typedef const __attribute__((address_space(1))) void* gp_t;
     typedef __attribute__((address_space(3))) void* lp_t;
     reinterpret_cast<f32x4*>(img)[tid] = f32x4{0.f, 0.f, 0.f, 0.f};
     reinterpret_cast<f32x4*>(img)[tid + kThreads] = f32x4{0.f, 0.f, 0.f, 0.f};
     const int zrow = tid >> 3, zg = tid & 7;
-    const f32x4 ev = *reinterpret_cast<const f32x4*>(reinterpret_cast<const float*>(w.aux0) + (size_t)min(m0 + zrow, w.M - 1) * w.ldx + min(4 * zg, w.ldx - 4));
-    const int t_i = wave & 1, t_c0 = (2 * ts + (wave >> 1)) * 32, t_sl = 2 * w.tail_kt;
+    const f32x4 ev = *reinterpret_cast<const f32x4*>(as_global(d.aux) + (size_t)min(zrow, d.mrem - 1) * d.ldx + min(4 * zg, d.ldx - 4));
+    const int t_i = wave & 1, t_c0 = (2 * ts + (wave >> 1)) * 32, t_sl = 2 * (int)(d.tk & 0xFF);
     u32x4 tb[TSL][2];
 #pragma unroll
     for (int j = 0; j < 2; ++j) {
-        const unsigned char* pw = reinterpret_cast<const unsigned char*>(w.tail_w) + (size_t)min(t_c0 + 16 * j + fr, w.tail_n - 1) * w.tail_ldw * ES + fq * 16;
+        const unsigned char* pw = as_global(d.tail_w) + (size_t)min(t_c0 + 16 * j + fr, d.tail_n - 1) * d.tail_ldw * ES + fq * 16;
 #pragma unroll
         for (int sl = 0; sl < TSL; ++sl) if (TSL == 2 || sl < t_sl) tb[sl][j] = *reinterpret_cast<const u32x4*>(pw + 64 * sl);
     }
     const int prow = wave * 8 + (lane >> 3), lc = ((lane & 7) ^ ((prow >> 1) & 7)) * 16;
-    const unsigned char* srcA = reinterpret_cast<const unsigned char*>(w.A) + (size_t)(m0 + prow) * w.lda * ES + lc;
-    const unsigned char* srcB = reinterpret_cast<const unsigned char*>(w.B) + (size_t)prow * w.ldb * ES + lc;
-    const size_t b32 = (size_t)32 * w.ldb * ES;
+    const unsigned char* srcA = d.a + (size_t)prow * d.lda * ES + lc;
+    const unsigned char* srcB = d.b + (size_t)prow * d.ldb * ES + lc;
+    const size_t b32 = (size_t)32 * d.ldb * ES;
 #define AVAE_H_DMA(kt, buf)                                                                                             \
     { __builtin_amdgcn_global_load_lds((gp_t)(srcA + (size_t)(kt) * kTileBytesK), (lp_t)(smem + (buf) * kHeadStage + wave * 1024), 16, 0, 0);       \
       __builtin_amdgcn_global_load_lds((gp_t)(srcB + (size_t)(kt) * kTileBytesK), (lp_t)(smem + (buf) * kHeadStage + (4 + wave) * 1024), 16, 0, 0); \
@@ -1674,6 +1765,7 @@
     AVAE_STAMP(1)
     const int npro = nk < RING - 1 ? nk : RING - 1;
     for (int p = 0; p < npro; ++p) AVAE_H_DMA(p, p)
+    behind_prologue();
     const int sw0 = (fq ^ (fr >> 1)) * 16;
     const int aoff = (wr * 16 + fr) * kTileBytesK, boff = (32 + wc * 32 + fr) * kTileBytesK;
     f32x4 acc[2] = {{0.f, 0.f, 0.f, 0.f}, {0.f, 0.f, 0.f, 0.f}};
@@ -1700,9 +1792,9 @@
     lds_barrier();
     AVAE_STAMP(3)
     {
-        const int orow = m0 + wr * 16 + fr, lrow = wr * 16 + fr;
-        float* mulv = reinterpret_cast<float*>(w.out0) + (size_t)orow * w.ld0;
-        const bool store = ts == 0 && orow < w.M;
+        const int lrow = wr * 16 + fr;
+        float* mulv = as_global(reinterpret_cast<float*>(d.out0)) + (size_t)lrow * d.ld0;
+        const bool store = ts == 0 && lrow < d.mrem;
 #pragma unroll
         for (int j = 0; j < 2; ++j) {
             const int c0 = wc * 32 + j * 16 + 4 * fq;
@@ -1716,15 +1808,15 @@
     lds_barrier();
     AVAE_STAMP(5)
     {
-        CT* Z = reinterpret_cast<CT*>(w.out1) + (size_t)(m0 + zrow) * w.ld1;
-        const bool store = ts == 0 && m0 + zrow < w.M;
+        CT* Z = as_global(reinterpret_cast<CT*>(d.out1)) + (size_t)zrow * d.ld1;
+        const bool store = ts == 0 && zrow < d.mrem;
 #pragma unroll
         for (int e = 0; e < 4; ++e) {
-            const int d = 4 * zg + e;
-            if (d < nz) {
-                const float z = __builtin_fmaf(fexp(0.5f * MV[zrow * LDM + nz + d]), ev[e], MV[zrow * LDM + d]);
-                img_put<CT>(img, zrow, d, z);
-                if (store) Z[d] = to_ct<CT>(z);
+            const int dim = 4 * zg + e;
+            if (dim < nz) {
+                const float z = __builtin_fmaf(fexp(0.5f * MV[zrow * LDM + nz + dim]), ev[e], MV[zrow * LDM + dim]);
+                img_put<CT>(img, zrow, dim, z);
+                if (store) Z[dim] = to_ct<CT>(z);
             }
         }
         if (tid < 32) img_put<CT>(img, tid, nz, 1.0f);
@@ -1741,9 +1833,63 @@
                 mma<CT>(tb[sl][0], ta, tacc[0][0]);
                 mma<CT>(tb[sl][1], ta, tacc[0][1]);
             }
-        regep_store<CT, 1, 2>(tacc, reinterpret_cast<CT*>(w.tail_out), w.tail_ldo, w.M, w.tail_n, m0 + arow, t_c0, lane,
+        regep_store<CT, 1, 2>(tacc, as_global(reinterpret_cast<CT*>(d.tail_out)), d.tail_ldo, d.mrem, d.tail_n, arow, t_c0, lane,
             [&](int, int, int, float v) { return act_fwd_t<ACT>(v); });
     }
+}
+
+template <typename CT, int ACT>
+__global__ void __launch_bounds__(kThreads) k_small_head(const LaunchArgs args, unsigned long long* stamps, int launch_id) {
+    constexpr int ES = (int)sizeof(CT);
+    unsigned char* smem = avae_dyn_smem;
+#ifdef AVAE_STAMPS
+    unsigned long long sv[kStampWords] = {0, 0, 0, 0, 0, 0, 0, 0};
+#endif
+    AVAE_STAMP(0)
+    const int part = blockIdx.x & 7, idx = blockIdx.x >> 3;
+    const WorkItem w = args.items[blockIdx.y];
+    asm volatile("" :: "s"(w.A), "s"(w.B), "s"(w.out0), "s"(w.out1), "s"(w.aux0), "s"(w.lda), "s"(w.ldb), "s"(w.K), "s"(w.ld0), "s"(w.tail_w), "s"(w.tail_out));
+    int t;
+    {
+        const int nt = w.tiles_m * w.tiles_n;
+        const int q = nt >> 3, r = nt & 7;
+        if (idx >= q + (part < r ? 1 : 0)) return;
+        t = (part < r ? part * (q + 1) : r * (q + 1) + (part - r) * q) + idx;
+    }
+    const int tm = t / w.tiles_n, ts = t - tm * w.tiles_n;
+    const int m0 = tm * 32;
+    HeadRec d;
+    d.a = reinterpret_cast<const unsigned char*>(w.A) + (size_t)m0 * w.lda * ES;
+    d.b = reinterpret_cast<const unsigned char*>(w.B);
+    d.out0 = reinterpret_cast<float*>(w.out0) + (size_t)m0 * w.ld0;
+    d.out1 = reinterpret_cast<CT*>(w.out1) + (size_t)m0 * w.ld1;
+    d.aux = reinterpret_cast<const float*>(w.aux0) + (size_t)m0 * w.ldx;
+    d.tail_w = reinterpret_cast<const unsigned char*>(w.tail_w);
+    d.tail_out = reinterpret_cast<CT*>(w.tail_out) + (size_t)m0 * w.tail_ldo;
+    d.lda = w.lda; d.ldb = w.ldb; d.ld0 = w.ld0; d.ld1 = w.ld1; d.ldx = w.ldx;
+    d.tail_ldw = w.tail_ldw; d.tail_ldo = w.tail_ldo;
+    d.nk = (w.K * ES) / kTileBytesK; d.nz = w.nz;
+    d.mrem = w.M - m0; d.tail_n = w.tail_n;
+    d.tk = HeadRec::pack(w.tail_kt, ts);
+    small_head_tile<CT, ACT>(d, []() {}, smem, AVAE_SV);
+    AVAE_STAMP(4)
+    AVAE_STAMP_FLUSH()
+}
+
+template <typename CT, int ACT>
+__global__ void __launch_bounds__(kThreads) k_head_rec(const HeadRec* __restrict__ tab, unsigned long long* stamps, int launch_id,
+                                                       const void* warm_lines, int warm_n) {
+    unsigned char* smem = avae_dyn_smem;
+#ifdef AVAE_STAMPS
+    unsigned long long sv[kStampWords] = {0, 0, 0, 0, 0, 0, 0, 0};
+#endif
+    AVAE_STAMP(0)
+    const HeadRec d = tab[blockIdx.x];
+    asm volatile("" :: "s"(d.a), "s"(d.b), "s"(d.out0), "s"(d.out1), "s"(d.aux), "s"(d.tail_w), "s"(d.tail_out), "s"(d.lda), "s"(d.ldb), "s"(d.ld0),
+                 "s"(d.ld1), "s"(d.ldx), "s"(d.tail_ldw), "s"(d.tail_ldo), "s"(d.nk), "s"(d.nz), "s"(d.mrem), "s"(d.tail_n), "s"(d.tk));
+    unsigned warmed = 0;
+    small_head_tile<CT, ACT>(d, [&]() { warmed = desc_warm(warm_lines, warm_n, __builtin_amdgcn_readfirstlane(threadIdx.x >> 6)); }, smem, AVAE_SV);
+    asm volatile("" :: "s"(warmed));
     AVAE_STAMP(4)
     AVAE_STAMP_FLUSH()
 }
@@ -1797,12 +1943,36 @@
 #undef K_LATB_B
 #undef K_LATB_F
 }
-
-#ifdef AVAE_STAMPS
-#define AVAE_SV sv
-#else
-#define AVAE_SV nullptr
-#endif
+#define AVAE_ACT_SWITCH(act, K, ...)                                                         \
+    switch (act) {                                                                           \
+        case AVAE_ACT_RELU: AVAE_LAUNCH((K(AVAE_ACT_RELU)), __VA_ARGS__); break;             \
+        case AVAE_ACT_SOFTPLUS: AVAE_LAUNCH((K(AVAE_ACT_SOFTPLUS)), __VA_ARGS__); break;     \
+        case AVAE_ACT_SIGMOID: AVAE_LAUNCH((K(AVAE_ACT_SIGMOID)), __VA_ARGS__); break;       \
+        case AVAE_ACT_TANH: AVAE_LAUNCH((K(AVAE_ACT_TANH)), __VA_ARGS__); break;             \
+        default: AVAE_LAUNCH((K(AVAE_ACT_IDENTITY)), __VA_ARGS__); break;                    \
+    }
+void launch_head_rec(int compute_dtype, int act, const HeadRec* tab, int n_recs, int lds_bytes, DescWarm warm, hipStream_t s,
+                     unsigned long long* stamps, int launch_id) {
+    const dim3 grid(n_recs), block(kThreads);
+#define K_HEAD_B(A) k_head_rec<__bf16, A>
+#define K_HEAD_F(A) k_head_rec<float, A>
+    if (compute_dtype == AVAE_BF16) { AVAE_ACT_SWITCH(act, K_HEAD_B, grid, block, lds_bytes, s, tab, stamps, launch_id, warm.lines, warm.n) }
+    else { AVAE_ACT_SWITCH(act, K_HEAD_F, grid, block, lds_bytes, s, tab, stamps, launch_id, warm.lines, warm.n) }
+#undef K_HEAD_B
+#undef K_HEAD_F
+}
+void launch_latb_rec(int compute_dtype, int act, const HeadRec* tab, int n_recs, int lds_bytes, DescWarm warm, DevState* st, const LaunchArgs& args,
+                     hipStream_t s, unsigned long long* stamps, int launch_id) {
+    const dim3 grid(n_recs), block(kThreads);
+#define K_LATB_B(A) k_latb_rec<__bf16, A>
+#define K_LATB_F(A) k_latb_rec<float, A>
+    if (compute_dtype == AVAE_BF16) { AVAE_ACT_SWITCH(act, K_LATB_B, grid, block, lds_bytes, s, tab, stamps, launch_id, warm.lines, warm.n, st, args) }
+    else { AVAE_ACT_SWITCH(act, K_LATB_F, grid, block, lds_bytes, s, tab, stamps, launch_id, warm.lines, warm.n, st, args) }
+#undef K_LATB_B
+#undef K_LATB_F
+}
+#undef AVAE_ACT_SWITCH
+
 template <typename CT, bool ADAM, typename F>
 __device__ __forceinline__ void small_tn_tile(const TnDesc& d, const TnDescArgs& ca, F&& behind_prologue, unsigned char* smem, unsigned long long* sv) {
     constexpr int BM = 64, RING = 4, ES = (int)sizeof(CT), EPR = kTileBytesK / ES, NCH = 4;
```

Result: faster. 5.062 million (median of 6 runs) (+1.5%).
